# chrished/DEMC.jl

Hardware: AMD Instinct MI355X
Metric: chain-updates/sec (N x gens/s) + gens-to-Rhat<1.05, MvNormal d=5 N=1024 (higher is better)
Workload: dtype f64

## Files before the change

### demc.jl_amd/_lib.py

```python
from __future__ import annotations

import ctypes as C
import os
import subprocess
from pathlib import Path

import numpy as np

PKG_DIR = Path(__file__).resolve().parent
REPO_ROOT = PKG_DIR.parent
LIB_PATH = Path(os.environ["DEMCZ_LIB"]) if os.environ.get("DEMCZ_LIB") else PKG_DIR / "libdemcz_hip.so"
ABI_VERSION = 1
LAYOUT_SPLIT = 100
LAYOUT_SPLIT_WAVE = 164
LAYOUT_PROGRAM_WAVE = 264

TARGET_MVNORMAL, TARGET_ISO_QUAD, TARGET_LINREG_SSE, TARGET_HOST_CALLBACK, TARGET_PROGRAM = 0, 1, 2, 3, 4
OK, ERR_INVALID_ARGUMENT, ERR_HIP, ERR_CAPACITY, ERR_STATE, ERR_NO_DEVICE, ERR_COMM = range(7)

_dp = C.POINTER(C.c_double)
_ip = C.POINTER(C.c_int32)
_lp = C.POINTER(C.c_int64)

SYMBOLS = [
    "demcz_abi_version", "demcz_create", "demcz_destroy", "demcz_last_error", "demcz_set_state",
    "demcz_get_state", "demcz_set_history_origin", "demcz_run", "demcz_synchronize",
    "demcz_get_history", "demcz_get_changed", "demcz_rhat", "demcz_accept_ratio", "demcz_mean_cov",
    "demcz_propose", "demcz_accept_commit", "demcz_end_generation", "demcz_comm_unique_id",
    "demcz_comm_init", "demcz_export_current_device", "demcz_append_rows_device",
    "demcz_set_external_append", "demcz_get_info", "demcz_selftest_draws", "demcz_append_rows",
    "demcz_rhat_partial", "demcz_set_rng_offset", "demcz_rhat_array", "demcz_accept_ratio_array",
    "demcz_mean_cov_array", "demcz_set_append_lag", "demcz_run_checked", "demcz_set_kernel_timing",
    "demcz_get_kernel_time", "demcz_set_live_spin_limit", "demcz_get_live_status",
    "demcz_debug_append_slab", "demcz_get_changed_total", "demcz_debug_set_live_fault",
    "demcz_set_comm_timeout", "demcz_debug_stall_exchange", "demcz_get_kernel_time_series",
    "demcz_history_stream", "demcz_get_history_view", "demcz_detach_history", "demcz_release_host_buffer", "demcz_get_archive_pinned",
    "demcz_debug_kernel_counts", "demcz_pool_trim", "demcz_debug_kernel_name", "demcz_peer_group", "demcz_get_peer_status", "demcz_peer_export", "demcz_peer_attach",
    "demcz_peer_detach", "demcz_get_peer_ping", "demcz_set_live_rearms", "demcz_get_live_rearms",
    "demcz_closure_buffers", "demcz_program_check", "demcz_set_program",
    "demcz_program_check_layout",
]


class DemczError(RuntimeError):
    def __init__(self, code: int, msg: str):
        super().__init__(f"libdemcz_hip status {code}: {msg}")
        self.code = code


class Config(C.Structure):
    _fields_ = [
        ("N", C.c_int64), ("chain_id0", C.c_int64), ("d", C.c_int32), ("K", C.c_int32),
        ("Mcap", C.c_int64), ("Gcap", C.c_int64), ("Nblocks", C.c_int32),
        ("block_offsets", _ip), ("block_indices", _ip), ("eps_scale", _dp),
        ("seed", C.c_uint64), ("device_id", C.c_int32), ("target_kind", C.c_int32),
        ("mu", _dp), ("W", _dp), ("c0", C.c_double), ("design", _dp), ("yobs", _dp),
        ("nobs", C.c_int64), ("stream", C.c_void_p), ("lanes_per_chain", C.c_int32),
        ("reserved0", C.c_int32),
    ]


HIPCC_FLAGS = ["-O3", "--offload-arch=gfx950", "-ffp-contract=off", "-fPIC", "-Werror", "-Wno-pass-failed"]


def sources() -> list:
    csrc = PKG_DIR / "csrc"
    return ([csrc / "demcz_capi.hip"] + sorted(csrc.glob("demcz_pw_inst_*.hip")) + sorted(csrc.glob("demcz_mlr_inst_*.hip"))
            + [csrc / "demcz_program.hip"])


def build_command(out: Path = LIB_PATH) -> list:
    return ["hipcc"] + HIPCC_FLAGS + ["-shared", "-o", str(out)] + [str(p) for p in sources()] + ["-lrccl", "-lhiprtc"]


def build_lib(out: Path = LIB_PATH, extra: list = (), jobs: int = 0) -> Path:
    from concurrent.futures import ThreadPoolExecutor
    objdir = REPO_ROOT / "build" / "obj" / Path(out).stem
    objdir.mkdir(parents=True, exist_ok=True)
    srcs = sources()
    jobs = jobs or max(1, min(len(srcs), len(os.sched_getaffinity(0))))

    def compile_one(src):
        obj = objdir / (src.stem + ".o")
        r = subprocess.run(["hipcc"] + list(extra) + HIPCC_FLAGS + ["-c", "-o", str(obj), str(src)], capture_output=True, text=True)
        if r.returncode != 0:
            raise RuntimeError(f"hipcc failed on {src.name}:\n{r.stderr[-4000:]}")
        return obj

    with ThreadPoolExecutor(max_workers=jobs) as ex:
        objs = list(ex.map(compile_one, srcs))
    subprocess.run(["hipcc", "--offload-arch=gfx950", "-shared", "-fPIC", "-o", str(out)] + [str(o) for o in objs] + ["-lrccl", "-lhiprtc"], check=True)
    return Path(out)


def build(force: bool = False) -> Path:
    srcs = list((PKG_DIR / "csrc").glob("*")) + [REPO_ROOT / "include" / "demcz.h"]
    if not force and LIB_PATH.exists():
        newest = max(p.stat().st_mtime for p in srcs)
        if LIB_PATH.stat().st_mtime >= newest:
            return LIB_PATH
    return build_lib(LIB_PATH)


_LIB = None


def load():
    global _LIB
    if _LIB is not None:
        return _LIB
    if not LIB_PATH.exists():
        raise FileNotFoundError(
            f"{LIB_PATH} is missing: build it with `python -c 'import __graft_entry__ as g; g.build()'` "
            "(hipcc --offload-arch=gfx950).  There is no CPU fallback.")
    L = C.CDLL(str(LIB_PATH))
    L.demcz_abi_version.restype = C.c_int32
    if L.demcz_abi_version() != ABI_VERSION:
        raise RuntimeError("libdemcz_hip.so ABI version mismatch: rebuild")
    L.demcz_last_error.restype = C.c_char_p
    L.demcz_last_error.argtypes = [C.c_void_p]
    L.demcz_create.argtypes = [C.POINTER(C.c_void_p), C.POINTER(Config)]
    L.demcz_destroy.argtypes = [C.c_void_p]
    L.demcz_set_state.argtypes = [C.c_void_p, _dp, _dp, _dp, C.c_int64, C.c_int64]
    L.demcz_get_state.argtypes = [C.c_void_p, _dp, _dp, _dp, C.c_int64, _lp]
    L.demcz_set_history_origin.argtypes = [C.c_void_p, C.c_int64]
    L.demcz_run.argtypes = [C.c_void_p, C.c_int64, C.c_int64, C.c_double, _dp]
    L.demcz_synchronize.argtypes = [C.c_void_p]
    L.demcz_get_history.argtypes = [C.c_void_p, C.c_int64, C.c_int64, _dp, _dp]
    L.demcz_get_changed.argtypes = [C.c_void_p, C.c_int64, C.c_int64, _lp]
    L.demcz_get_changed_total.argtypes = [C.c_void_p, C.c_int64, C.c_int64, _lp, _ip]
    L.demcz_rhat.argtypes = [C.c_void_p, C.c_int64, C.c_int64, _dp]
    L.demcz_accept_ratio.argtypes = [C.c_void_p, C.c_int64, C.c_int64, _dp]
    L.demcz_mean_cov.argtypes = [C.c_void_p, C.c_int64, C.c_int64, _dp, _dp]
    L.demcz_propose.argtypes = [C.c_void_p, C.c_int64, C.c_int32, C.c_double, _dp]
    L.demcz_accept_commit.argtypes = [C.c_void_p, _dp, _dp]
    L.demcz_end_generation.argtypes = [C.c_void_p, C.c_int64]
    L.demcz_closure_buffers.argtypes = [C.c_void_p, C.POINTER(C.c_void_p), C.POINTER(C.c_void_p)]
    L.demcz_comm_unique_id.argtypes = [C.c_void_p]
    L.demcz_comm_init.argtypes = [C.c_void_p, C.c_void_p, C.c_int32, C.c_int32]
    L.demcz_export_current_device.argtypes = [C.c_void_p, C.c_void_p]
    L.demcz_append_rows_device.argtypes = [C.c_void_p, C.c_void_p, C.c_int64, C.c_int64]
    L.demcz_append_rows.argtypes = [C.c_void_p, _dp, C.c_int64, C.c_int64]
    L.demcz_rhat_partial.argtypes = [C.c_void_p, C.c_int64, C.c_int64, C.c_int32, _dp, _dp]
    L.demcz_set_rng_offset.argtypes = [C.c_void_p, C.c_int64]
    L.demcz_set_append_lag.argtypes = [C.c_void_p, C.c_int32]
    L.demcz_rhat_array.argtypes = [C.c_int32, _dp, C.c_int64, C.c_int32, C.c_int64, _dp]
    L.demcz_accept_ratio_array.argtypes = [C.c_int32, _dp, C.c_int64, C.c_int64, _dp]
    L.demcz_mean_cov_array.argtypes = [C.c_int32, _dp, C.c_int64, C.c_int32, C.c_int64, _dp, _dp]
    L.demcz_set_external_append.argtypes = [C.c_void_p, C.c_int32]
    L.demcz_get_info.argtypes = [C.c_void_p, _lp, _lp, _ip]
    L.demcz_selftest_draws.argtypes = [C.c_int32, C.c_uint64, C.c_uint64, C.c_uint64, C.c_int32,
                                       C.POINTER(C.c_uint64), _dp, _dp]
    L.demcz_set_live_spin_limit.argtypes = [C.c_void_p, C.c_int32]
    L.demcz_get_live_status.argtypes = [C.c_void_p, _ip, _ip]
    L.demcz_debug_kernel_counts.argtypes = [C.c_void_p, _lp]
    L.demcz_history_stream.argtypes = [C.c_void_p, C.c_int32]
    L.demcz_get_history_view.argtypes = [C.c_void_p, C.c_int64, C.c_int64, C.POINTER(C.c_void_p), C.POINTER(C.c_void_p)]
    L.demcz_detach_history.argtypes = [C.c_void_p, C.POINTER(C.c_void_p), C.POINTER(C.c_void_p)]
    L.demcz_release_host_buffer.argtypes = [C.c_void_p]
    L.demcz_pool_trim.argtypes = [_lp, _lp]
    L.demcz_peer_group.argtypes = [C.POINTER(C.c_void_p), C.c_int32]
    L.demcz_get_peer_status.argtypes = [C.c_void_p, _ip, _ip]
    L.demcz_peer_export.argtypes = [C.c_void_p, C.c_int32, C.c_int32, C.c_void_p]
    L.demcz_peer_attach.argtypes = [C.c_void_p, C.c_void_p]
    L.demcz_peer_detach.argtypes = [C.c_void_p]
    L.demcz_get_peer_ping.argtypes = [C.c_void_p, _ip, _dp]
    L.demcz_set_live_rearms.argtypes = [C.c_void_p, C.c_int32]
    L.demcz_get_live_rearms.argtypes = [C.c_void_p, _ip, _ip]
    L.demcz_debug_kernel_name.argtypes = [C.c_void_p, C.c_char_p, C.c_int32]
    L.demcz_program_check.argtypes = [C.c_int32, C.c_char_p, C.c_char_p]
    L.demcz_program_check_layout.argtypes = [C.c_int32, C.c_char_p, C.c_char_p, C.c_int32]
    L.demcz_set_program.argtypes = [C.c_void_p, C.c_char_p, C.c_char_p, _dp, C.c_int64]
    L.demcz_get_archive_pinned.argtypes = [C.c_void_p, C.POINTER(C.c_void_p), _lp]
    L.demcz_get_kernel_time_series.argtypes = [C.c_void_p, C.c_int32, _dp, _dp, _ip]
    L.demcz_set_comm_timeout.argtypes = [C.c_void_p, C.c_int64]
    L.demcz_debug_stall_exchange.argtypes = [C.c_void_p, C.c_int32]
    L.demcz_debug_set_live_fault.argtypes = [C.c_void_p, C.c_int32, C.c_int64]
    L.demcz_debug_append_slab.argtypes = [C.c_void_p, _dp, C.c_int32, C.c_int32, C.c_int32]
    for name in SYMBOLS:
        fn = getattr(L, name)
        if name != "demcz_last_error":
            fn.restype = C.c_int32
    _LIB = L
    return L


def f64(a, order="C"):
    return np.require(a, dtype=np.float64, requirements=["F" if order == "F" else "C", "A"])


def ptr(a, t=_dp):
    return a.ctypes.data_as(t) if a is not None else None
```

### demc.jl_amd/csrc/demcz_capi.hip

```cpp
#include "../../include/demcz.h"
#include "demcz_kernels.h"
#include "demcz_kernels_ml.h"
#include "demcz_kernels_pc.h"
#include "demcz_kernels_lr.h"
#include "demcz_kernels_ps.h"
#include "demcz_kernels_ps2.h"
#include "demcz_kernels_ps2d.h"
#include "demcz_pw_dispatch.h"
#include "demcz_mlr_dispatch.h"
#include "demcz_program.h"

#include <rccl/rccl.h>

#include <algorithm>
#include <chrono>
#include <thread>
#include <cstdlib>
#include <deque>
#include <mutex>
#include <cmath>
#include <cstdio>
#include <cstring>
#include <string>
#include <unordered_map>
// ... 123 lines not shown
    bool steady = false;
    KernelArm arm = ARM_ONE_LANE;
    bool live = false, temper = false;
    int pw_form = 0;
};

struct LaunchFacts {
    bool live = false;
    bool temper = false;
    bool ps2 = false;
    bool dual = false;
    bool pw_reg = false;
    bool pw_matrix = false;
    bool coop = false;
    bool lr16 = false;
};

struct PeerGroup {
    std::vector<demcz_handle*> members;
    bool failed = false;
    int32_t rearms_left = 3;
    bool lockstep_only = false;
    bool busy = false;
    bool dead = false;
};

struct demcz_handle {
    demcz_config cfg{};
    int lanes = 1;
    hipStream_t stream = nullptr;
    bool own_stream = false;
    std::string err;
    std::vector<int32_t> block_offsets, block_indices, slot_of;
    std::vector<double> eps;
    int64_t S = 0;
    int64_t ZS = 0;
    bool full_block = false;
    int ngrp = 1;
    uint64_t gstart = 1ull;
    int mlb_qb = 0;
    double* dZ = nullptr;
    double* dX = nullptr;
    double* dlp = nullptr;
    double* dchain = nullptr;
    double* dchain_alloc = nullptr;
    double* dlogobj = nullptr;
    double* dlp_origin = nullptr;
    bool origin_valid = false;
    double* dtemp = nullptr;
    int64_t temp_cap = 0;
    int32_t* d_block_offsets = nullptr;
    int32_t* d_slot_of = nullptr;
    double* d_eps = nullptr;
    double* d_mu = nullptr;
    double* d_Wp = nullptr;
    double* d_design = nullptr;
    double* d_y = nullptr;
    double* d_scratch = nullptr;
    int64_t scratch_cap = 0;
    double* d_stage = nullptr;
    int64_t stage_cap = 0;
    int64_t M = 0;
    int64_t g_done = 0;
    int64_t g0 = 0;
    int64_t rng_offset = 0;
    bool has_state = false;
    int64_t launches = 0;
    mutable int64_t kernel_counts[1] = {0};
    WindowKernel last_kernel;
    bool external_append = false;
    double* dXprop = nullptr;
    double* dlogu = nullptr;
    bool proposal_pending = false;
    bool gen_open = false;
    double* hc_X = nullptr;
    double* hc_lp = nullptr;
    volatile unsigned int* hc_flag = nullptr;
    unsigned int* hc_count = nullptr;
    unsigned int hc_seq = 0;
    hipStream_t diag_stream = nullptr;
    hipEvent_t diag_ev = nullptr;
    hipEvent_t rhat_side_ev = nullptr;
    bool rhat_side_pending = false;
    double* d_spec_X = nullptr;
    double* d_spec_lp = nullptr;
    hipEvent_t spec_ev = nullptr;
    double* pinned_rhat = nullptr;
    unsigned int* pinned_err = nullptr;
    int64_t pinned_err_launches = -1;
    int64_t pinned_cap = 0;
    bool timing = false;
    std::vector<std::pair<hipEvent_t, hipEvent_t>> timed;
    std::vector<double> series_start_ms, series_dur_ms;
    int64_t timed_launches = 0;
    int64_t live_wg_cap = -1;
    SplitKind split_kind = SPLIT_NONE;
    int split_lanes = 0;
    int split_per_wg = 1;
    int32_t* d_slot_role = nullptr;
    double* d_rec[2] = {nullptr, nullptr};
    unsigned int* d_live_err = nullptr;
#ifdef DEMCZ_STAMPS
    unsigned long long* d_stamps = nullptr;
#endif
    bool arena = false, rec_in_arena = false, hist_joint = false;
    int64_t arena_gens = 0;
    double* arena_rec[2] = {nullptr, nullptr};
    double* arena_temp = nullptr;
    int64_t rec_cap = 0;
    int rec_cur = 0;
    bool host_paced = false;
    int wpw = 1;
    bool ps_dual = false;
    bool dual_now = false;
    bool lr_spec = false;
    bool no_live = false;
    bool live_claimed = false;
    unsigned int live_spin_limit = 0;
    int32_t live_fault_polls = 0;
    int64_t live_fault_g = 0;
    bool in_checked = false;
    struct RunCall { int64_t g_from, g_to; double gamma; bool tempered; std::vector<double> temperature; };
    std::vector<RunCall> live_log;
    double* d_safe_X = nullptr;
    double* d_safe_lp = nullptr;
    bool snap_pending = false;
    int64_t safe_M = 0, safe_M_app = 0, safe_g_done = 0;
    bool replaying = false;
    int32_t live_redos = 0;
    int32_t live_rearms_left = 3;
    int32_t live_rearms = 0;
    int64_t rearm_from = -1;
    uint32_t fail_row_hint = 0xffffffffu;
    struct RecDesc { bool valid = false; int64_t g_first = 0, M = 0, rows = 0; int32_t ngen = 0, boff = 0; } rec_desc[2];
    hipStream_t prod_stream = nullptr;
    hipEvent_t prod_done[2] = {nullptr, nullptr};
    hipEvent_t prod_gate = nullptr;
    bool prod_pending[2] = {false, false};
    hipEvent_t after_launch_ev = nullptr;
    unsigned int* d_acc = nullptr;
    int64_t acc_waves = 0;
    int32_t acc_slots = 0, acc_next = 0;
    struct LaunchRec { int64_t g_first, g_last; int32_t slot; };
    std::deque<LaunchRec> acc_log;
    ncclComm_t comm = nullptr;
    ncclComm_t comm_side = nullptr;
    int nranks = 1, rank = 0;
    double* d_gather = nullptr;
    int lag = 0;
    int64_t M_app = 0;
    struct PendingRows { int64_t visible_from; int64_t M_after; hipEvent_t ev; int64_t xseq = 0; };
    std::deque<PendingRows> pending;
    int64_t batch_J = -1;
    hipStream_t comm_stream = nullptr;
    double* d_send[2] = {nullptr, nullptr};
    double* d_recv[2] = {nullptr, nullptr};
    hipEvent_t buf_done[2] = {nullptr, nullptr};
    int64_t xseq = 0, xseq_waited = 0, buf_xseq[2] = {0, 0};
    int batch_buf = 0, batch_cnt = 0;
    int64_t batch_base = 0;
    bool hs_on = false;
    double* hs_chain = nullptr;
    double* hs_logobj = nullptr;
    hipStream_t hs_stream = nullptr;
    bool pooled_dev = false;
    volatile long long* xdone = nullptr;
// ... 673 lines not shown
        for (int r = 0; r < DEMCZ_MAX_PEERS; ++r)
            if (h->ipc_mapped[r]) { (void)hipIpcCloseMemHandle(h->ipc_mapped[r]); h->ipc_mapped[r] = nullptr; }
        if (met) {
            met = false;
            if (ncclAllReduce(h->d_err_all + 1, h->d_err_all + 1, 1, ncclUint32, ncclMax, h->comm, h->stream) == ncclSuccess)
                met = sync_stream(h, h->stream, "demcz_destroy (peers, mappings closed)") == DEMCZ_OK;
        }
        if (!met && h->archive_fine) h->dZ = nullptr;
    }
    h->n_peers = 0;
    h->peer_mode = 0;
}

extern "C" int32_t demcz_destroy(demcz_handle* h)
{
    if (!h) return DEMCZ_OK;
    (void)hipSetDevice(h->cfg.device_id);
    for (hipStream_t st : {h->stream, h->prod_stream, h->diag_stream, h->comm_stream, h->hs_stream})
        if (st && !h->comm_dead) (void)sync_stream(h, st, "demcz_destroy");
    peer_detach(h);
    live_release(h);
    free_all(h);
    delete h;
    return DEMCZ_OK;
}

static TargetParams target_params(const demcz_handle* h)
{
    TargetParams tp;
    tp.mu = h->d_mu; tp.Wp = h->d_Wp; tp.c0 = h->cfg.c0;
    tp.design = h->d_design; tp.yobs = h->d_y; tp.nobs = h->cfg.nobs;
    tp.ngrp = h->ngrp; tp.goff = h->d_block_offsets; tp.gstart = h->gstart;
    return tp;
}

static int32_t ensure_scratch(demcz_handle* h, int64_t n)
{
    if (n <= h->scratch_cap) return DEMCZ_OK;
    { int32_t rcq = quiesce_all(h); if (rcq) return rcq; }
    SYNCCHK(h, h->stream);
    if (h->diag_stream) SYNCCHK(h, h->diag_stream);
    if (h->prod_stream) SYNCCHK(h, h->prod_stream);
    if (h->d_scratch) HIPCHK(h, dev_free(h->cfg.device_id, h->d_scratch));
    h->d_scratch = nullptr; h->scratch_cap = 0;
    HIPCHK(h, dev_malloc(h->cfg.device_id, (void**)&h->d_scratch, (size_t)n * sizeof(double)));
    h->scratch_cap = n;
    return DEMCZ_OK;
}

static int32_t launch_logp(demcz_handle* h, const double* X, int64_t ldX, int64_t n, double* out)
{
    const TargetParams tp = target_params(h);
    const int bs = 64;
    const dim3 grid((unsigned)((n + bs - 1) / bs));
    switch (h->cfg.target_kind) {
    case DEMCZ_TARGET_MVNORMAL:
        hipLaunchKernelGGL(logp_kernel<TARGET_MVNORMAL>, grid, dim3(bs), 0, h->stream, tp, h->cfg.d, X, ldX, n, out); break;
    case DEMCZ_TARGET_ISO_QUAD:
        hipLaunchKernelGGL(logp_kernel<TARGET_ISO_QUAD>, grid, dim3(bs), 0, h->stream, tp, h->cfg.d, X, ldX, n, out); break;
    case DEMCZ_TARGET_LINREG_SSE:
        hipLaunchKernelGGL(logp_kernel<TARGET_LINREG_SSE>, grid, dim3(bs), 0, h->stream, tp, h->cfg.d, X, ldX, n, out); break;
    case DEMCZ_TARGET_PROGRAM: {
        if (!h->prog_ready) return fail(h, DEMCZ_ERR_STATE, "program target: call demcz_set_program first");
        TargetParams tpv = tp;
        int dv = h->cfg.d;
        void* args[] = {&tpv, &dv, &X, &ldX, &n, &out};
        HIPCHK(h, hipModuleLaunchKernel(h->prog.logp, grid.x, 1, 1, bs, 1, 1, 0, h->stream, args, nullptr));
        break;
    }
    default: return fail(h, DEMCZ_ERR_STATE, "host-callback target: pass logp explicitly");
    }
    HIPCHK(h, hipGetLastError());
    return DEMCZ_OK;
}

extern "C" int32_t demcz_set_state(demcz_handle* h, const double* X, const double* logp, const double* Z,
                                   int64_t ldZ, int64_t M0)
{
    if (!h) return DEMCZ_ERR_INVALID_ARGUMENT;
    DEADCHK(h);
    if (!X || !Z) return fail(h, DEMCZ_ERR_INVALID_ARGUMENT, "demcz_set_state: X and Z are required");
    if (M0 < 2) return fail(h, DEMCZ_ERR_INVALID_ARGUMENT, "demcz_set_state: M0 >= 2 needed (two distinct archive rows, demcz.jl:176-179)");
    if (M0 > h->cfg.Mcap || ldZ < M0) return fail(h, DEMCZ_ERR_CAPACITY, "demcz_set_state: M0 exceeds Mcap or ldZ < M0");
    if (!logp && h->cfg.target_kind == DEMCZ_TARGET_HOST_CALLBACK)
        return fail(h, DEMCZ_ERR_INVALID_ARGUMENT, "demcz_set_state: host-callback target needs logp");
    if (h->cfg.target_kind == DEMCZ_TARGET_PROGRAM && !h->prog_ready)
        return fail(h, DEMCZ_ERR_STATE, "demcz_set_state: program target: call demcz_set_program first");
    HIPCHK(h, hipSetDevice(h->cfg.device_id));
    const int d = h->cfg.d;
    const int64_t N = h->cfg.N;
    HIPCHK(h, hipMemcpyAsync(h->dX, X, (size_t)N * d * sizeof(double), hipMemcpyHostToDevice, h->stream));
    {
        int32_t rcz = ensure_scratch(h, M0 * d);
        if (rcz) return rcz;
        HIPCHK(h, hipMemcpy2DAsync(h->d_scratch, (size_t)M0 * sizeof(double), Z, (size_t)ldZ * sizeof(double),
                                   (size_t)M0 * sizeof(double), (size_t)d, hipMemcpyHostToDevice, h->stream));
        const int64_t tot = M0 * d;
        hipLaunchKernelGGL(append_rows_kernel, dim3((unsigned)((tot + 255) / 256)), dim3(256), 0, h->stream, h->dZ, h->ZS,
                           (int64_t)0, (const double*)h->d_scratch, M0, M0, d);
        HIPCHK(h, hipGetLastError());
        const size_t rest = (size_t)(h->cfg.Mcap - M0) * (size_t)h->ZS;
        if (rest > 0) {
            hipLaunchKernelGGL(fill_u64_kernel, dim3((unsigned)((rest + 255) / 256)), dim3(256), 0, h->stream,
                               reinterpret_cast<unsigned long long*>(h->dZ + (size_t)M0 * h->ZS), rest, LIVE_SENTINEL);
            HIPCHK(h, hipGetLastError());
        }
        HIPCHK(h, hipMemsetAsync(h->d_live_err, 0, 4 * sizeof(unsigned int), h->stream));
    }
    if (logp) {
        HIPCHK(h, hipMemcpyAsync(h->dlp, logp, (size_t)N * sizeof(double), hipMemcpyHostToDevice, h->stream));
    } else {
        int32_t rc = launch_logp(h, h->dX, N, N, h->dlp);
        if (rc) return rc;
    }
    HIPCHK(h, hipMemcpyAsync(h->dlp_origin, h->dlp, (size_t)N * sizeof(double), hipMemcpyDeviceToDevice, h->stream));
    SYNCCHK(h, h->stream);
    h->M = M0;
    h->M_app = M0;
    h->peer_fence = true;
    if (h->no_live && h->rearm_from >= 0) h->rearm_from = 0;
    h->live_log.clear();
    h->snap_pending = false;
    h->acc_log.clear();
    { int32_t rcs = rec_scrub(h); if (rcs) return rcs; }
    for (auto& pe : h->pending) if (pe.ev) (void)hipEventDestroy(pe.ev);
    h->pending.clear();
    h->batch_cnt = 0; h->batch_J = -1;
    h->g_done = h->g0;
    h->origin_valid = true;
    h->has_state = true;
    h->proposal_pending = false;
    h->gen_open = false;
    return DEMCZ_OK;
}

extern "C" int32_t demcz_get_state(demcz_handle* h, double* X, double* logp, double* Z, int64_t ldZ, int64_t* M)
{
    if (!h) return DEMCZ_ERR_INVALID_ARGUMENT;
    DEADCHK(h);
    if (!h->has_state) return fail(h, DEMCZ_ERR_STATE, "demcz_get_state: no state set");
    HIPCHK(h, hipSetDevice(h->cfg.device_id));
    {
        int32_t rcv = live_verify(h);
        if (rcv) return rcv;
    }
    const int d = h->cfg.d;
    const int64_t N = h->cfg.N;
    if (X) HIPCHK(h, hipMemcpyAsync(X, h->dX, (size_t)N * d * sizeof(double), hipMemcpyDeviceToHost, h->stream));
    if (logp) HIPCHK(h, hipMemcpyAsync(logp, h->dlp, (size_t)N * sizeof(double), hipMemcpyDeviceToHost, h->stream));
    if (Z) {
        const int64_t Mall = h->M_app;
        if (ldZ < Mall) return fail(h, DEMCZ_ERR_INVALID_ARGUMENT, "demcz_get_state: ldZ < M");
        int32_t rcz = flush_exchanges(h);
        if (rcz) return rcz;
        rcz = ensure_scratch(h, Mall * d);
        if (rcz) return rcz;
        const int64_t tot = Mall * d;
        hipLaunchKernelGGL(export_rows_kernel, dim3((unsigned)((tot + 255) / 256)), dim3(256), 0, h->stream, (const double*)h->dZ,
                           h->ZS, (int64_t)0, h->d_scratch, Mall, Mall, d);
        HIPCHK(h, hipGetLastError());
        HIPCHK(h, hipMemcpy2DAsync(Z, (size_t)ldZ * sizeof(double), h->d_scratch, (size_t)Mall * sizeof(double),
                                   (size_t)Mall * sizeof(double), (size_t)d, hipMemcpyDeviceToHost, h->stream));
    }
    SYNCCHK(h, h->stream);
    if (M) *M = h->M_app;
    return DEMCZ_OK;
// ... 111 lines not shown
    if (h->cfg.target_kind == DEMCZ_TARGET_PROGRAM && !h->prog_ready)
        return fail(h, DEMCZ_ERR_STATE, "demcz_run: program target: call demcz_set_program first");
    if (!k.fn && !k.mod) return fail(h, DEMCZ_ERR_STATE, "window launch: target / dimension not built for this handle's layout");
    void* args[] = {const_cast<WindowParams*>(&P)};
    if (k.mod) {
        HIPCHK(h, hipModuleLaunchKernel(k.mod, (unsigned)blocks, 1, 1, (unsigned)k.threads, 1, 1, (unsigned)k.dyn_lds, h->stream, args, nullptr));
    } else {
        allow_dynamic_lds(h->cfg.device_id, k);
        HIPCHK(h, hipLaunchKernel(k.fn, dim3((unsigned)blocks), dim3((unsigned)k.threads), args, k.dyn_lds, h->stream));
    }
    HIPCHK(h, hipGetLastError());
    if (k.steady) ++h->kernel_counts[0];
    return DEMCZ_OK;
}

static int ml_lanes_available(int target_kind, int d, bool full_block, int64_t nobs, int max_blocklen = 0, int nblocks = 1)
{
    if (!full_block) {
        if (nblocks > MLB_MAX_BLOCKS) return 0;
        if (target_kind == DEMCZ_TARGET_MVNORMAL) {
            if ((d == 5 || d == 6 || d == 10) && 2 + (max_blocklen + 1) / 2 <= 8) return 8;
            if (d == 20 && 2 + (max_blocklen + 1) / 2 <= 16) return 16;
        }
        return 0;
    }
    if (target_kind == DEMCZ_TARGET_LINREG_SSE && d == 10 &&
        lr16_dynamic_lds<10>(nobs) <= ML_MAX_DYNAMIC_LDS)
        return 16;
    if (target_kind == DEMCZ_TARGET_LINREG_SSE && d >= 2 && d <= 28) return 16;
    if (target_kind == DEMCZ_TARGET_MVNORMAL) {
        if (d >= 2 && d <= 10) return 8;
        if (d == 20) return 16;
    }
    if (target_kind == DEMCZ_TARGET_ISO_QUAD && d == 10) return 8;
    return 0;
}

static bool mlb32_wanted(int64_t)
{
    static const char* env = getenv("DEMCZ_MLB_L32");
    return env && atoi(env) != 0;
}

static bool pc_available(int target_kind, int d, bool full_block)
{
    if (!full_block) return false;
    if (target_kind == DEMCZ_TARGET_ISO_QUAD) return d == 10;
    return target_kind == DEMCZ_TARGET_MVNORMAL && d >= 2 && d <= 10;
}

static bool split_ml_available(int target_kind, int d, bool full_block, int64_t nobs)
{
    if (!full_block) return false;
    if (target_kind == DEMCZ_TARGET_MVNORMAL) return d == 20;
    return target_kind == DEMCZ_TARGET_LINREG_SSE && d == 10 && lr16_dynamic_lds<10>(nobs) <= ML_MAX_DYNAMIC_LDS;
}

static bool ps_available(int target_kind, int d)
{
    if (target_kind == DEMCZ_TARGET_MVNORMAL) return d >= 2 && d <= PW_D_MAX;
    return target_kind == DEMCZ_TARGET_ISO_QUAD && d >= PW_D_MIN && d <= PW_D_MAX;
}

static int pc_roles(int d) { return ((d == 1) ? 1 : (d + 1) / 2) + 2; }
static int64_t rec_fields(const demcz_handle* h) { return (h->split_kind == SPLIT_MLB) ? 2 * h->S : (int64_t)h->cfg.d + 2; }
static int64_t rec_roles(const demcz_handle* h) { return (h->split_kind == SPLIT_MLB) ? h->S : pc_roles(h->cfg.d); }

#ifdef DEMCZ_STAMPS
constexpr int64_t DEMCZ_STAMP_WGS = 1 << 16;
#endif

static bool pw_matrix_form(const demcz_handle* h)
{
    const char* on = getenv("DEMCZ_PW_MFMA");
    return on && atoi(on) != 0 && h->cfg.d == 20 && h->cfg.target_kind == DEMCZ_TARGET_MVNORMAL;
}

static bool pw_regular(const WindowParams& P, bool live)
{
    static const bool no_reg = getenv("DEMCZ_NO_PW_REG") != nullptr;
    return live && !no_reg && P.K % PS_R == 0 && P.to_boundary % PS_R == 0 && P.ngen % PS_R == 0 && P.ngen >= PS_R;
}

static int32_t launch_window_pc(demcz_handle* h, const WindowParams& P, const WindowKernel& k, bool live = false)
{
    const int64_t nbc = (P.N + 63) / 64;
    const bool pc_records = !(h->split_kind == SPLIT_MLB);
    const int64_t units = pc_records ? produce_units(P.N, (int)rec_roles(h), P.rec_fields, P.next_ngen) : nbc * rec_roles(h) * P.next_ngen;
    const int upw = k.waves;
    const int64_t blocks = P.consumer_blocks + (units + upw - 1) / upw;
    if (blocks <= 0) return DEMCZ_OK;
    if (h->split_kind == SPLIT_WAVE || h->lr_spec) {
        if (h->split_kind == SPLIT_WAVE && P.ZS != ((P.d <= 2) ? 2 : (P.d <= 4) ? 4 : ((P.d + 7) / 8) * 8)) return fail(h, DEMCZ_ERR_STATE, "split layout: archive row stride");
        const int bin = (P.rec_in == h->d_rec[0]) ? 0 : 1, bout = (P.rec_out == h->d_rec[0]) ? 0 : 1;
        const bool one_launch = !live && P.consumer_blocks > 0;
        if (units > 0 && one_launch && h->prod_pending[bout]) {
            HIPCHK(h, hipStreamWaitEvent(h->stream, h->prod_done[bout], 0));
            h->prod_pending[bout] = false;
        }
        if (units > 0 && !one_launch) {
            hipStream_t ps = h->stream;
            static const bool serial_env = getenv("DEMCZ_PRODUCE_SERIAL") != nullptr;
            if (P.consumer_blocks > 0 && !serial_env && h->peer_mode != 1) {
                if (!h->prod_stream) {
                    HIPCHK(h, stream_acquire(h->cfg.device_id, &h->prod_stream));
                    HIPCHK(h, hipEventCreateWithFlags(&h->prod_gate, hipEventDisableTiming));
                    for (int b = 0; b < 2; ++b) HIPCHK(h, hipEventCreateWithFlags(&h->prod_done[b], hipEventDisableTiming));
                }
                if (h->after_launch_ev) {
                    HIPCHK(h, hipStreamWaitEvent(h->prod_stream, h->after_launch_ev, 0));
                } else {
                    HIPCHK(h, hipEventRecord(h->prod_gate, h->stream));
                    HIPCHK(h, hipStreamWaitEvent(h->prod_stream, h->prod_gate, 0));
                }
                ps = h->prod_stream;
            } else if (h->prod_pending[bout]) {
                HIPCHK(h, hipStreamWaitEvent(h->stream, h->prod_done[bout], 0));
                h->prod_pending[bout] = false;
            }
            const dim3 pg((unsigned)((units + PRODUCE_WAVES - 1) / PRODUCE_WAVES)), pw(64 * PRODUCE_WAVES);
            static const size_t throttle_env = getenv("DEMCZ_PRODUCE_LDS") ? (size_t)atol(getenv("DEMCZ_PRODUCE_LDS")) : PRODUCE_THROTTLE_LDS;
            size_t big_d = throttle_env;
            if (h->split_kind == SPLIT_WAVE && P.d > 20) {
                int plds = 0;
                if (h->prog_wave && (!h->prog_ready || hipFuncGetAttribute(&plds, HIP_FUNC_ATTRIBUTE_SHARED_SIZE_BYTES, h->prog.wave[1][0]) != hipSuccess)) plds = (int)ML_MAX_DYNAMIC_LDS;
                size_t clds = (size_t)plds;
                if (!h->prog_wave) {
                    WindowKernel lk[MAX_LIVE_KERNELS];
                    const int nlk = live_kernels(h, lk);
                    for (int i = 0; i < nlk; ++i) {
                        hipFuncAttributes a{};
                        if (lk[i].fn && hipFuncGetAttributes(&a, lk[i].fn) == hipSuccess) clds = std::max(clds, (size_t)a.sharedSizeBytes);
                    }
                }
                const size_t room = (clds + 4096 < ML_MAX_DYNAMIC_LDS) ? ML_MAX_DYNAMIC_LDS - clds - 4096 : 8192;
                big_d = std::max<size_t>(8192, std::min<size_t>(throttle_env, room));
            }
            const size_t dyn = (ps != h->stream) ? (h->lr_spec ? (size_t)8192 : (h->ps_dual && !getenv("DEMCZ_PRODUCE_LDS")) ? (size_t)32768 : big_d) : 0;
            switch (P.d) {
#define DEMCZ_PRODUCE_CASE(DD) case DD: hipLaunchKernelGGL((produce_kernel<DD>), pg, pw, dyn, ps, P); break;
            DEMCZ_PRODUCE_CASE(2) DEMCZ_PRODUCE_CASE(3) DEMCZ_PRODUCE_CASE(4) DEMCZ_PRODUCE_CASE(5) DEMCZ_PRODUCE_CASE(6) DEMCZ_PRODUCE_CASE(7)
            DEMCZ_PRODUCE_CASE(8) DEMCZ_PRODUCE_CASE(9) DEMCZ_PRODUCE_CASE(10) DEMCZ_PRODUCE_CASE(11) DEMCZ_PRODUCE_CASE(12) DEMCZ_PRODUCE_CASE(13)
            DEMCZ_PRODUCE_CASE(14) DEMCZ_PRODUCE_CASE(15) DEMCZ_PRODUCE_CASE(16) DEMCZ_PRODUCE_CASE(17) DEMCZ_PRODUCE_CASE(18) DEMCZ_PRODUCE_CASE(19)
            DEMCZ_PRODUCE_CASE(20) DEMCZ_PRODUCE_CASE(21) DEMCZ_PRODUCE_CASE(22) DEMCZ_PRODUCE_CASE(23) DEMCZ_PRODUCE_CASE(24) DEMCZ_PRODUCE_CASE(25)
            DEMCZ_PRODUCE_CASE(26) DEMCZ_PRODUCE_CASE(27) DEMCZ_PRODUCE_CASE(28) DEMCZ_PRODUCE_CASE(29) DEMCZ_PRODUCE_CASE(30) DEMCZ_PRODUCE_CASE(31)
            DEMCZ_PRODUCE_CASE(32)
#undef DEMCZ_PRODUCE_CASE
            default: return fail(h, DEMCZ_ERR_STATE, "split layout: dimension not built");
            }
            HIPCHK(h, hipGetLastError());
            if (ps != h->stream) {
                HIPCHK(h, hipEventRecord(h->prod_done[bout], ps));
                h->prod_pending[bout] = true;
            }
        }
        if (P.consumer_blocks > 0) {
            if (h->prod_pending[bin]) {
                if (h->host_paced) { int32_t rcw = sync_event(h, h->prod_done[bin], "launch_window_pc"); if (rcw) return rcw; }
                else HIPCHK(h, hipStreamWaitEvent(h->stream, h->prod_done[bin], 0));
                h->prod_pending[bin] = false;
            }
            static_assert(PS_CHAINS == LR16_WAVES, "producer units per workgroup of a one-launch grid");
            const int64_t grid = P.consumer_blocks + (one_launch ? (units + PS_CHAINS - 1) / PS_CHAINS : 0);
            return launch_kernel(h, k, grid, P);
        }
        return DEMCZ_OK;
    }
    return launch_kernel(h, k, blocks, P);
}

static int32_t rec_reserve(demcz_handle* h, int64_t gens)
{
    if (gens <= h->rec_cap) return DEMCZ_OK;
    { int32_t rcq = quiesce_all(h); if (rcq) return rcq; }
    SYNCCHK(h, h->stream);
    if (h->prod_stream) SYNCCHK(h, h->prod_stream);
    h->prod_pending[0] = h->prod_pending[1] = false;
    if (h->arena && gens <= h->arena_gens && h->rec_cap == 0) {
        for (int b = 0; b < 2; ++b) { h->d_rec[b] = h->arena_rec[b]; h->rec_desc[b].valid = false; }
        h->rec_in_arena = true;
        h->rec_cap = h->arena_gens;
        return DEMCZ_OK;
    }
    for (int b = 0; b < 2; ++b) {
        if (h->d_rec[b] && !h->rec_in_arena) HIPCHK(h, dev_free(h->cfg.device_id, h->d_rec[b]));
        h->d_rec[b] = nullptr;
        const size_t nd = (size_t)gens * (size_t)rec_fields(h) * h->cfg.N + REC_PAD;
        HIPCHK(h, dev_malloc(h->cfg.device_id, (void**)&h->d_rec[b], nd * sizeof(double)));
        HIPCHK(h, hipMemsetAsync(h->d_rec[b], 0, nd * sizeof(double), h->stream));
        h->rec_desc[b].valid = false;
    }
    h->rec_in_arena = false;
    h->rec_cap = gens;
    return DEMCZ_OK;
}

static bool ps2_applicable(const demcz_handle* h, const WindowParams& P)
{
    static const bool off = getenv("DEMCZ_NO_PS2") != nullptr;
    if (off || h->split_kind != SPLIT_WAVE || h->prog_wave || P.d < 2 || P.d > 5 || !h->arena || !h->rec_in_arena) return false;
    if (P.temperature && (P.temperature < h->arena_temp || P.temperature >= h->arena_temp + h->arena_gens)) return false;
    if (P.K % PS2_R != 0 || P.to_boundary % PS2_R != 0 || P.ngen % PS2_R != 0 || P.ngen < PS2_R) return false;
    if (P.chain && (!h->hist_joint || (double)h->cfg.N * (h->cfg.d + 1) * (double)h->cfg.Gcap * 8.0 >= 4293918720.0)) return false;
    return true;
}

static int32_t pc_prepare(demcz_handle* h, WindowParams& P, int64_t cur_rows, int64_t next_g, int64_t next_ngen, int64_t next_M,
                          int64_t next_rows, int32_t next_boff)
{
    {
        int32_t rcr = rec_reserve(h, std::max<int64_t>(P.ngen, next_ngen));
        if (rcr) return rcr;
    }
    P.rec_stride = h->rec_cap;
    const int cur = h->rec_cur;
    const int32_t cur_boff = P.K - P.to_boundary;
    auto& dc = h->rec_desc[cur];
    if (!(dc.valid && dc.g_first == P.g_first && dc.ngen >= P.ngen && dc.M == P.M && dc.rows == cur_rows && dc.boff == cur_boff)) {
        WindowParams Q = P;
        Q.consumer_blocks = 0;
        Q.rec_out = h->d_rec[cur];
        Q.next_g_first = P.g_first; Q.next_ngen = P.ngen; Q.next_M = P.M; Q.next_rows = cur_rows; Q.next_boff = cur_boff;
        int32_t rc = launch_window_pc(h, Q, window_kernel_of(h, launch_facts(h, &Q, false)));
        if (rc) return rc;
        dc.valid = true; dc.g_first = P.g_first; dc.M = P.M; dc.ngen = P.ngen; dc.rows = cur_rows; dc.boff = cur_boff;
    }
    P.rec_in = h->d_rec[cur];
    const int per_wg = (h->ps_dual && !h->dual_now) ? PS_CHAINS : h->split_per_wg;
    P.consumer_blocks = (int32_t)((P.N + per_wg - 1) / per_wg);
    P.rec_out = h->d_rec[cur ^ 1];
    P.next_g_first = next_g; P.next_ngen = (int32_t)std::max<int64_t>(next_ngen, 0); P.next_M = next_M;
    P.next_rows = next_rows; P.next_boff = next_boff;
    auto& dn = h->rec_desc[cur ^ 1];
    dn.valid = next_ngen > 0; dn.g_first = next_g; dn.M = next_M; dn.ngen = (int32_t)std::max<int64_t>(next_ngen, 0);
    dn.rows = next_rows; dn.boff = next_boff;
    h->rec_cur = cur ^ 1;
// ... 282 lines not shown
    if (h->batch_cnt == 0) return DEMCZ_OK;
    const int d = h->cfg.d, cnt = h->batch_cnt, buf = h->batch_buf;
    const int64_t N = h->cfg.N;
    hipEvent_t ready;
    HIPCHK(h, hipEventCreateWithFlags(&ready, hipEventDisableTiming));
    HIPCHK(h, hipEventRecord(ready, h->stream));
    HIPCHK(h, hipStreamWaitEvent(h->comm_stream, ready, 0));
    HIPCHK(h, hipEventDestroy(ready));
    { int32_t rcs = maybe_stall(h, h->comm_stream); if (rcs) return rcs; }
    NCCLCHK(h, ncclAllGather(h->d_send[buf], h->d_recv[buf], (size_t)N * d * cnt, ncclDouble, h->comm_side, h->comm_stream));
    const int64_t tot = N * d * cnt * h->nranks;
    hipLaunchKernelGGL(append_batch_kernel, dim3((unsigned)((tot + 255) / 256)), dim3(256), 0, h->comm_stream, h->dZ, h->ZS,
                       h->batch_base, (const double*)h->d_recv[buf], N, h->nranks, cnt, d);
    HIPCHK(h, hipGetLastError());
    hipEvent_t done;
    HIPCHK(h, hipEventCreateWithFlags(&done, hipEventDisableTiming));
    HIPCHK(h, hipEventRecord(done, h->comm_stream));
    h->pending.back().ev = done;
    h->pending.back().xseq = ++h->xseq;
    if (!h->xdone) {
        HIPCHK(h, host_malloc((void**)&h->xdone, sizeof(long long)));
        *h->xdone = 0;
    }
    hipLaunchKernelGGL(mark_kernel, dim3(1), dim3(1), 0, h->comm_stream, h->xdone, (long long)h->xseq);
    HIPCHK(h, hipGetLastError());
    h->buf_xseq[buf] = h->xseq;
    HIPCHK(h, hipEventRecord(h->buf_done[buf], h->comm_stream));
    h->batch_cnt = 0;
    h->batch_buf ^= 1;
    h->batch_J = -1;
    return DEMCZ_OK;
}

static int32_t admit_pending(demcz_handle* h, int64_t g)
{
    while (!h->pending.empty() && h->pending.front().visible_from <= g) {
        auto pe = h->pending.front();
        if (pe.ev) {
            if (h->host_paced && h->xdone) {
                volatile long long* xd = h->xdone;
                const long long need = (long long)pe.xseq;
                int32_t rcw = wait_deadline(h, [xd, need]() { return (*xd >= need) ? hipSuccess : hipErrorNotReady; }, "admit_pending (exchange of a batch)");
                if (rcw) return rcw;
            }
            else HIPCHK(h, hipStreamWaitEvent(h->stream, pe.ev, 0));
            HIPCHK(h, hipEventDestroy(pe.ev));
            h->xseq_waited = std::max(h->xseq_waited, pe.xseq);
        }
        h->M = pe.M_after;
        h->pending.pop_front();
    }
    return DEMCZ_OK;
}

static int32_t flush_exchanges(demcz_handle* h)
{
    if (h->comm && h->lag > 0) {
        int32_t rc = exchange_batch(h);
        if (rc) return rc;
        for (auto& pe : h->pending)
            if (pe.ev) HIPCHK(h, hipStreamWaitEvent(h->stream, pe.ev, 0));
    }
    return DEMCZ_OK;
}

static int32_t check_live_err(demcz_handle* h)
{
    unsigned int e[4] = {0, 0, 0, 0};
    if (!h->d_live_err) return DEMCZ_OK;
    if (h->err_clean) return DEMCZ_OK;
    HIPCHK(h, hipMemcpy(e, h->d_live_err, sizeof(e), hipMemcpyDeviceToHost));
    if (!e[0]) h->err_clean = true;
    if (e[0])
        return fail(h, DEMCZ_ERR_HIP, "demcz_run: an archive row appended inside the launch never became visible (LIVE hand-off): "
                                      "generation " + std::to_string(e[1]) + " of the launch, row " + std::to_string(e[2]) +
                                      ", workgroup " + std::to_string(e[3]) + ", rows appended " + std::to_string(h->M_app));
    return DEMCZ_OK;
}

static int32_t live_rollback(demcz_handle* h, std::vector<demcz_handle::RunCall>& calls)
{
    calls.swap(h->live_log);
    h->live_log.clear();
    const int64_t N = h->cfg.N;
    const int d = h->cfg.d;
    SYNCCHK(h, h->stream);
    if (h->diag_stream) SYNCCHK(h, h->diag_stream);
    if (h->prod_stream) SYNCCHK(h, h->prod_stream);
    if (!h->snap_pending) {
        HIPCHK(h, hipMemcpyAsync(h->dX, h->d_safe_X, (size_t)N * d * sizeof(double), hipMemcpyDeviceToDevice, h->stream));
        HIPCHK(h, hipMemcpyAsync(h->dlp, h->d_safe_lp, (size_t)N * sizeof(double), hipMemcpyDeviceToDevice, h->stream));
    }
    h->snap_pending = false;
    if (h->M_app > h->safe_M_app) {
        const size_t rest = (size_t)(h->M_app - h->safe_M_app) * (size_t)h->ZS;
        hipLaunchKernelGGL(fill_u64_kernel, dim3((unsigned)((rest + 255) / 256)), dim3(256), 0, h->stream,
                           reinterpret_cast<unsigned long long*>(h->dZ + (size_t)h->safe_M_app * h->ZS), rest, LIVE_SENTINEL);
        HIPCHK(h, hipGetLastError());
    }
    HIPCHK(h, hipMemsetAsync(h->d_live_err, 0, 4 * sizeof(unsigned int), h->stream));
    SYNCCHK(h, h->stream);
    h->peer_fence = true;
    int64_t from = h->g_done;
    if (h->fail_row_hint != 0xffffffffu && (int64_t)h->fail_row_hint >= h->safe_M_app && (int64_t)h->fail_row_hint < h->M_app) {
        const int64_t rows = h->cfg.N * ((h->comm || h->peer_mode != 0) ? h->nranks : 1);
        const int64_t j = ((int64_t)h->fail_row_hint - h->safe_M_app) / rows;
        from = std::min<int64_t>(from, (h->safe_g_done / h->cfg.K + 1 + j) * (int64_t)h->cfg.K + 1);
    }
    h->fail_row_hint = 0xffffffffu;
    h->M = h->safe_M;
    h->M_app = h->safe_M_app;
    h->g_done = h->safe_g_done;
    while (!h->acc_log.empty() && h->acc_log.back().g_last > h->safe_g_done) h->acc_log.pop_back();
    { int32_t rcs = rec_scrub(h); if (rcs) return rcs; }
    h->no_live = true;
    h->rearm_from = -1;
    if (h->peer_mode != 1 && h->peer_mode != 3 && h->live_rearms_left > 0) {
        --h->live_rearms_left;
        h->rearm_from = from;
    }
    h->live_fault_polls = 0;
    live_release(h);
    ++h->live_redos;
    return DEMCZ_OK;
}

static int32_t live_try_rearm(demcz_handle* h)
{
    h->rearm_from = -1;
    h->no_live = false;
    unsigned int ok = live_span(h) > 0 ? 1u : 0u;
    if (h->peer_mode == 2 && h->comm && h->d_err_all) {
        HIPCHK(h, hipMemcpyAsync(h->d_err_all + 2, &ok, sizeof(ok), hipMemcpyHostToDevice, h->stream));
        NCCLCHK(h, ncclAllReduce(h->d_err_all + 2, h->d_err_all + 2, 1, ncclUint32, ncclMin, h->comm, h->stream));
        SYNCCHK(h, h->stream);
        HIPCHK(h, hipMemcpy(&ok, h->d_err_all + 2, sizeof(ok), hipMemcpyDeviceToHost));
    }
    if (!ok) {
        h->no_live = true;
        live_release(h);
        return DEMCZ_OK;
    }
    ++h->live_rearms;
    if (getenv("DEMCZ_DEBUG_LIVE")) fprintf(stderr, "[demcz] rank %d: LIVE launches re-armed (%d re-arms left)\n", h->rank, (int)h->live_rearms_left);
    return DEMCZ_OK;
}

static int32_t live_failed(demcz_handle* h, bool& failed)
{
    failed = false;
    SYNCCHK(h, h->stream);
    unsigned int e[4] = {0, 0, 0, 0};
    if (h->peer_mode == 2 && !h->no_live && h->comm) {
        NCCLCHK(h, ncclAllReduce(h->d_live_err, h->d_err_all, 1, ncclUint32, ncclMax, h->comm, h->stream));
        SYNCCHK(h, h->stream);
        HIPCHK(h, hipMemcpy(e, h->d_err_all, sizeof(unsigned int), hipMemcpyDeviceToHost));
    } else if (h->pinned_err && h->pinned_err_launches == h->launches) {
        std::memcpy(e, h->pinned_err, sizeof(e));
    } else {
        HIPCHK(h, hipMemcpy(e, h->d_live_err, sizeof(e), hipMemcpyDeviceToHost));
    }
    h->pinned_err_launches = -1;
    failed = e[0] != 0u;
    if (!failed && h->peer_mode != 2) h->err_clean = true;
    if (failed) {
        unsigned int row = 0xffffffffu;
// ... 322 lines not shown

extern "C" int32_t demcz_run(demcz_handle* h, int64_t g_from, int64_t g_to, double gamma, const double* temperature)
{
    if (!h) return DEMCZ_ERR_INVALID_ARGUMENT;
    DEADCHK(h);
    if (!h->has_state) return fail(h, DEMCZ_ERR_STATE, "demcz_run: call demcz_set_state first");
    if (g_from < 1 || g_to < g_from) return fail(h, DEMCZ_ERR_INVALID_ARGUMENT, "demcz_run: need 1 <= g_from <= g_to");
    if (h->cfg.target_kind == DEMCZ_TARGET_HOST_CALLBACK)
        return fail(h, DEMCZ_ERR_STATE, "demcz_run: host-callback target uses demcz_propose/accept_commit");
    const bool hist = h->cfg.Gcap > 0;
    if (hist && (g_from - h->g0 - 1 < 0 || g_to - h->g0 > h->cfg.Gcap))
        return fail(h, DEMCZ_ERR_CAPACITY, "demcz_run: generations outside the history window (demcz_set_history_origin)");
    HIPCHK(h, hipSetDevice(h->cfg.device_id));
    const int64_t G = g_to - g_from + 1;
    const int K = h->cfg.K;
    const bool sharded = (h->comm != nullptr);
    if (h->peer_mode == 1 && (!h->group || h->group->dead))
        return fail(h, DEMCZ_ERR_STATE, "demcz_run: a member of this handle's replica group has been destroyed");
    if (h->no_live && h->rearm_from >= 0 && g_from > h->rearm_from) {
        int32_t rcr = live_try_rearm(h);
        if (rcr) return rcr;
    }
    const bool peer = h->peer_mode != 0 && live_span(h) > 0;
    const bool rccl_exchange = sharded && !peer;
    const bool kernel_appends = !rccl_exchange && !h->external_append;
    const int64_t shards = (sharded || h->peer_mode != 0) ? h->nranks : 1;
    {
        const int64_t nb = g_to / K - (g_from - 1) / K;
        const int64_t rows = h->cfg.N * shards;
        if (!h->external_append && h->M_app + nb * rows > h->cfg.Mcap)
            return fail(h, DEMCZ_ERR_CAPACITY, "demcz_run: Z row capacity (Mcap) would be exceeded");
        if (h->external_append && nb > 1)
            return fail(h, DEMCZ_ERR_STATE, "demcz_run: with external append a call may cross at most one K boundary, at its end");
        if (h->external_append && nb == 1 && (g_to % K) != 0)
            return fail(h, DEMCZ_ERR_STATE, "demcz_run: with external append the K boundary must be the last generation of the call");
    }
    if (h->peer_mode == 3 && h->peers_closed)
        return fail(h, DEMCZ_ERR_STATE, "demcz_run: the peers' archives have been closed (demcz_peer_detach): this handle runs no further generations");
    if (h->peer_mode == 3 && !peer)
        return fail(h, DEMCZ_ERR_STATE, "demcz_run: host-mediated IPC peers run with the in-launch hand-off only (it is not available: a timed-out "
                                        "hand-off, an append lag, caller-owned appends, or more chains than a LIVE launch holds)");
    if (h->peer_mode == 1 && !peer && !h->replaying) {
        if (h->lag != 0 || h->external_append) return fail(h, DEMCZ_ERR_STATE, "demcz_run: replica groups run with append lag 0 and library-owned appends");
        demcz_handle::RunCall rcall{g_from, g_to, gamma, temperature != nullptr, {}};
        if (temperature) rcall.temperature.assign(temperature, temperature + G);
        h->live_log.push_back(std::move(rcall));
        return DEMCZ_OK;
    }
    const bool temp_in_arena = temperature && h->arena && h->arena_temp && G <= h->arena_gens;
    if (temperature && temp_in_arena) {
        SYNCCHK(h, h->stream);
        HIPCHK(h, hipMemcpyAsync(h->arena_temp, temperature, (size_t)G * sizeof(double), hipMemcpyHostToDevice, h->stream));
        SYNCCHK(h, h->stream);
    } else if (temperature) {
        if (G > h->temp_cap) {
            { int32_t rcq = quiesce_all(h); if (rcq) return rcq; }
            SYNCCHK(h, h->stream);
            if (h->dtemp) HIPCHK(h, dev_free(h->cfg.device_id, h->dtemp));
            h->dtemp = nullptr; h->temp_cap = 0;
            HIPCHK(h, dev_malloc(h->cfg.device_id, (void**)&h->dtemp, (size_t)(G + 8) * sizeof(double)));
            HIPCHK(h, hipMemsetAsync(h->dtemp, 0, (size_t)(G + 8) * sizeof(double), h->stream));
            h->temp_cap = G;
        }
        HIPCHK(h, hipMemcpyAsync(h->dtemp, temperature, (size_t)G * sizeof(double), hipMemcpyHostToDevice, h->stream));
        SYNCCHK(h, h->stream);
    }
    WindowParams P;
    P.Z = h->dZ; P.Zw = h->dZ; P.ZS = h->ZS;
    P.Xcur = h->dX; P.lpcur = h->dlp;
    P.chain = hist ? h->dchain : nullptr; P.logobj = hist ? h->dlogobj : nullptr;
#ifdef DEMCZ_EXP_NOHIST
    P.chain = nullptr; P.logobj = nullptr;
#endif
    P.N = h->cfg.N; P.chain_id0 = h->cfg.chain_id0; P.d = h->cfg.d;
    P.gamma = gamma; P.seed = h->cfg.seed; P.S = h->S; P.Nblocks = h->cfg.Nblocks;
    P.block_offsets = h->d_block_offsets; P.slot_of = h->d_slot_of; P.eps = h->d_eps; P.slot_role = h->d_slot_role;
    P.tp = target_params(h);
    P.snap = nullptr;
    P.K = K;
    P.acc_out = nullptr; P.live_err = h->d_live_err; P.live_spin_limit = LIVE_SPIN_LIMIT;
    P.safe_X = nullptr; P.safe_lp = nullptr;
    P.rec_in = nullptr; P.rec_out = nullptr; P.next_g_first = 0; P.next_M = 0; P.next_ngen = 0; P.consumer_blocks = 0;
    P.next_rows = 0; P.next_boff = 0; P.rec_stride = 0;
    P.rec_fields = (h->lanes == DEMCZ_LAYOUT_SPLIT && h->split_kind == SPLIT_ML) ? h->cfg.d + 2 : 0;
    P.z_bytes = (uint32_t)std::min<size_t>(h->dZ_bytes, 0xffffffffull);
    P.hist_bytes = (hist && h->hist_joint) ? (uint32_t)std::min<double>((double)h->cfg.N * (h->cfg.d + 1) * (double)h->cfg.Gcap * 8.0, 4294967295.0) : 0u;
    P.brows = h->cfg.N * (peer ? shards : 1);
    P.row_off = peer ? (int64_t)h->rank * h->cfg.N : 0;
    P.n_peers = peer ? h->n_peers : 0;
    for (int r = 0; r < DEMCZ_MAX_PEERS; ++r) P.peer_Z[r] = (peer && r < h->n_peers) ? h->peer_Z[r] : nullptr;
    if (peer && h->peer_mode == 2 && h->peer_fence) {
        NCCLCHK(h, ncclAllReduce(h->d_err_all + 1, h->d_err_all + 1, 1, ncclUint32, ncclMax, h->comm, h->stream));
        h->peer_fence = false;
    }
#ifdef DEMCZ_STAMPS
    if (!h->d_stamps) {
        HIPCHK(h, dev_malloc(h->cfg.device_id, (void**)&h->d_stamps, (size_t)DEMCZ_STAMP_WGS * 16 * sizeof(unsigned long long)));
        HIPCHK(h, hipMemset(h->d_stamps, 0, (size_t)DEMCZ_STAMP_WGS * 16 * sizeof(unsigned long long)));
    }
    P.stamps = h->d_stamps;
#endif
    const int E = h->lag;
    int64_t g = g_from;
    if (h->lanes == DEMCZ_LAYOUT_SPLIT) {
        const int64_t lm = live_span(h);
        int64_t cap = (lm > 0) ? lm : (int64_t)K * std::max(E, 1);
        if (lm > 0 && hist) cap = std::max<int64_t>(std::min<int64_t>(cap, h->cfg.Gcap), std::min<int64_t>(cap, G));
        int32_t rcr = rec_reserve(h, cap);
        if (rcr) return rcr;
    }
    if (live_span(h) > 0) {
        if (h->live_log.size() >= 256 && !h->in_checked && !h->replaying && h->peer_mode != 1) {
            int32_t rcv = live_verify(h);
            if (rcv) return rcv;
        }
        if (live_span(h) > 0) {
            if (h->live_log.empty() && !h->replaying) {
                const int64_t N = h->cfg.N;
                const int d = h->cfg.d;
                if (!h->d_safe_X) HIPCHK(h, dev_malloc(h->cfg.device_id, (void**)&h->d_safe_X, (size_t)N * d * sizeof(double)));
                if (!h->d_safe_lp) HIPCHK(h, dev_malloc(h->cfg.device_id, (void**)&h->d_safe_lp, (size_t)N * sizeof(double)));
                if (h->live_fault_polls < 0) {
                    HIPCHK(h, hipMemsetAsync(h->d_safe_X, 0xff, (size_t)N * d * sizeof(double), h->stream));
                    HIPCHK(h, hipMemsetAsync(h->d_safe_lp, 0xff, (size_t)N * sizeof(double), h->stream));
                }
                h->snap_pending = true;
                h->safe_M = h->M; h->safe_M_app = h->M_app; h->safe_g_done = h->g_done;
            }
            demcz_handle::RunCall rcall{g_from, g_to, gamma, temperature != nullptr, {}};
            if (temperature) rcall.temperature.assign(temperature, temperature + G);
            h->live_log.push_back(std::move(rcall));
        }
    }
    struct EventPair {
        hipEvent_t a = nullptr, b = nullptr;
        ~EventPair() { if (a) (void)hipEventDestroy(a); if (b) (void)hipEventDestroy(b); }
    } tev;
    int64_t timed_launches = 0;
    const bool timed = h->timing && h->timed.size() < 4096;
    if (timed) {
        HIPCHK(h, hipEventCreate(&tev.a));
        HIPCHK(h, hipEventCreate(&tev.b));
        HIPCHK(h, hipEventRecord(tev.a, h->stream));
    }
    while (g <= g_to) {
        const int64_t next_boundary = ((g - 1) / K + 1) * K;
        int64_t w_end = std::min(next_boundary, g_to);
        if (E > 0 && !h->external_append) {
            const int64_t jn = next_boundary / K, J = ((jn + E - 1) / E) * E;
            w_end = std::min(J * (int64_t)K, g_to);
        }
        int64_t live_max = live_span(h);
        h->dual_now = false;
        if (h->ps_dual) {
            const int64_t tb0 = next_boundary - g + 1, rest = g_to - g + 1;
            const bool temp_ok = !temperature || temp_in_arena;
            const bool hist_ok = !hist || (double)h->cfg.N * (h->cfg.d + 1) * (double)h->cfg.Gcap * 8.0 < 4293918720.0;
            const bool reg = K % PS2_R == 0 && tb0 % PS2_R == 0 && rest >= PS2_R && temp_ok && hist_ok && h->arena && h->rec_in_arena;
            if (reg) {
                h->dual_now = true;
                if (live_max > 0) live_max = std::max<int64_t>((std::min(live_max, rest) / PS2_R) * PS2_R, PS2_R);
                else w_end = g + ((w_end - g + 1) / PS2_R) * PS2_R - 1;
            } else {
                live_max = 0;
            }
        }
// ... 208 lines not shown
        if (first >= 0 && r.g_last == g_to) { last = i; break; }
    }
    bool ok = first >= 0 && last >= first;
    for (int i = first; ok && i < last; ++i)
        ok = h->acc_log[i].g_last + 1 == h->acc_log[i + 1].g_first && (h->acc_log[i].slot + 1) % h->acc_slots == h->acc_log[i + 1].slot;
    if (ok && h->d_acc) {
        rc = ensure_scratch(h, 1);
        if (rc) return rc;
        static_assert(sizeof(long long) == sizeof(double), "scratch reuse");
        hipLaunchKernelGGL(sum_counts_kernel, dim3(1), dim3(256), 0, h->stream, (const unsigned int*)h->d_acc, h->acc_waves,
                           (int)h->acc_log[first].slot, last - first + 1, (int)h->acc_slots, skip, (long long*)h->d_scratch);
        HIPCHK(h, hipGetLastError());
        long long v = 0;
        HIPCHK(h, hipMemcpyAsync(&v, h->d_scratch, sizeof(v), hipMemcpyDeviceToHost, h->stream));
        SYNCCHK(h, h->stream);
        *total = (int64_t)v;
        if (from_ballots) *from_ballots = 1;
        return DEMCZ_OK;
    }
    std::vector<int64_t> ch((size_t)(g_to - g_from + 1));
    rc = demcz_get_changed(h, g_from, g_to, ch.data());
    if (rc) return rc;
    int64_t t = 0;
    for (int64_t v : ch) t += v;
    *total = t;
    if (from_ballots) *from_ballots = 0;
    return DEMCZ_OK;
}

struct RhatPlan { int64_t N, w, s0, n, nd; int d, nchunk; double *S1, *S2, *mean_j, *s2_j, *sums; };

static int32_t rhat_prepare(demcz_handle* h, int64_t g_from, int64_t g_to, RhatPlan& r, bool compute, hipStream_t qs = nullptr)
{
    int32_t rc = check_hist_range(h, g_from, g_to, "demcz_rhat");
    if (rc) return rc;
    r.N = h->cfg.N; r.w = g_to - g_from + 1; r.s0 = g_from - h->g0 - 1; r.d = h->cfg.d;
    r.n = r.w / 2;
    if (r.n < 2) return fail(h, DEMCZ_ERR_INVALID_ARGUMENT, "demcz_rhat: window needs at least 4 generations");
    HIPCHK(h, hipSetDevice(h->cfg.device_id));
    r.nchunk = (int)std::min<int64_t>(std::max<int64_t>(1, r.n / 32), 32);
    r.nd = r.N * r.d;
    const int64_t need = 2 * (2 * r.nchunk * r.nd) + 2 * (2 * r.nd) + 4 * r.d;
    rc = ensure_scratch(h, need);
    if (rc) return rc;
    r.S1 = h->d_scratch;
    r.S2 = r.S1 + 2 * r.nchunk * r.nd;
    r.mean_j = r.S2 + 2 * r.nchunk * r.nd;
    r.s2_j = r.mean_j + 2 * r.nd;
    r.sums = r.s2_j + 2 * r.nd;
    if (compute) {
        const int bs = 256;
        const unsigned gx = (unsigned)((r.nd + bs - 1) / bs);
        if (!qs) qs = h->stream;
        hipLaunchKernelGGL(rhat_moments_kernel, dim3(gx, 2 * r.nchunk), dim3(bs), 0, qs, h->dchain, r.N, r.d, r.s0, r.n, r.nchunk, r.S1, r.S2);
        hipLaunchKernelGGL(rhat_chainstats_kernel, dim3(gx, 2), dim3(bs), 0, qs, h->dchain, r.N, r.d, r.s0, r.n, r.nchunk, r.S1, r.S2, r.mean_j, r.s2_j);
        HIPCHK(h, hipGetLastError());
    }
    return DEMCZ_OK;
}

extern "C" int32_t demcz_rhat_partial(demcz_handle* h, int64_t g_from, int64_t g_to, int32_t stage, const double* grand, double* out)
{
    if (!h || !out || (stage != 0 && stage != 1) || (stage == 1 && !grand)) return DEMCZ_ERR_INVALID_ARGUMENT;
    RhatPlan r;
    int32_t rc = live_verify(h);
    if (rc) return rc;
    rc = rhat_prepare(h, g_from, g_to, r, true);
    if (rc) return rc;
    const int d = r.d;
    if (stage == 0) {
        hipLaunchKernelGGL(rhat_reduce_kernel, dim3(d), dim3(256), 0, h->stream, r.mean_j, r.s2_j, r.N, d, 0, (const double*)nullptr, 1.0, r.sums);
        HIPCHK(h, hipGetLastError());
        HIPCHK(h, hipMemcpyAsync(out, r.sums, (size_t)d * sizeof(double), hipMemcpyDeviceToHost, h->stream));
    } else {
        HIPCHK(h, hipMemcpyAsync(r.sums, grand, (size_t)d * sizeof(double), hipMemcpyHostToDevice, h->stream));
        hipLaunchKernelGGL(rhat_reduce_kernel, dim3(d), dim3(256), 0, h->stream, r.mean_j, r.s2_j, r.N, d, 1, (const double*)r.sums, 1.0, r.sums + d);
        HIPCHK(h, hipGetLastError());
        HIPCHK(h, hipMemcpyAsync(out, r.sums + d, (size_t)2 * d * sizeof(double), hipMemcpyDeviceToHost, h->stream));
    }
    SYNCCHK(h, h->stream);
    return DEMCZ_OK;
}

static int32_t rhat_enqueue(demcz_handle* h, int64_t g_from, int64_t g_to, double* out, bool side = false)
{
    RhatPlan r;
    hipStream_t qs = h->stream;
    static const bool own_env = getenv("DEMCZ_RHAT_OWN_STREAM") != nullptr;
    if (side && !h->comm && !own_env && h->prod_stream) {
        if (!h->diag_ev) HIPCHK(h, hipEventCreateWithFlags(&h->diag_ev, hipEventDisableTiming));
        if (h->after_launch_ev) {
            HIPCHK(h, hipStreamWaitEvent(h->prod_stream, h->after_launch_ev, 0));
        } else {
            HIPCHK(h, hipEventRecord(h->diag_ev, h->stream));
            HIPCHK(h, hipStreamWaitEvent(h->prod_stream, h->diag_ev, 0));
            h->after_launch_ev = h->diag_ev;
        }
        qs = h->prod_stream;
    } else if (side && h->comm && h->peer_mode == 2 && !h->no_live && h->comm_side && h->comm_stream && h->lag == 0) {
        if (!h->diag_ev) HIPCHK(h, hipEventCreateWithFlags(&h->diag_ev, hipEventDisableTiming));
        if (h->after_launch_ev) {
            HIPCHK(h, hipStreamWaitEvent(h->comm_stream, h->after_launch_ev, 0));
        } else {
            HIPCHK(h, hipEventRecord(h->diag_ev, h->stream));
            HIPCHK(h, hipStreamWaitEvent(h->comm_stream, h->diag_ev, 0));
            h->after_launch_ev = h->diag_ev;
        }
        qs = h->comm_stream;
    } else if (side && !h->comm) {
        if (!h->diag_stream) HIPCHK(h, stream_acquire(h->cfg.device_id, &h->diag_stream));
        if (!h->diag_ev) HIPCHK(h, hipEventCreateWithFlags(&h->diag_ev, hipEventDisableTiming));
        if (h->after_launch_ev) {
            HIPCHK(h, hipStreamWaitEvent(h->diag_stream, h->after_launch_ev, 0));
        } else {
            HIPCHK(h, hipEventRecord(h->diag_ev, h->stream));
            HIPCHK(h, hipStreamWaitEvent(h->diag_stream, h->diag_ev, 0));
            h->after_launch_ev = h->diag_ev;
        }
        qs = h->diag_stream;
    }
    if (qs == h->stream && h->rhat_side_pending) {
        HIPCHK(h, hipStreamWaitEvent(h->stream, h->rhat_side_ev, 0));
        h->rhat_side_pending = false;
    }
    struct SideMark {
        demcz_handle* h; hipStream_t qs;
        ~SideMark() {
            if (qs == h->stream) return;
            if (!h->rhat_side_ev && hipEventCreateWithFlags(&h->rhat_side_ev, hipEventDisableTiming) != hipSuccess) { h->rhat_side_ev = nullptr; return; }
            if (hipEventRecord(h->rhat_side_ev, qs) == hipSuccess) h->rhat_side_pending = true;
        }
    } side_mark{h, qs};
    int32_t rc = rhat_prepare(h, g_from, g_to, r, true, qs);
    if (rc) return rc;
    const int d = r.d;
    const int64_t n = r.n;
    const int64_t m = 2 * r.N * h->nranks;
    const bool sharded = (h->comm != nullptr);
    double* sums = r.sums;
    if (!sharded) {
        hipLaunchKernelGGL(rhat_tail_kernel, dim3(d), dim3(256), 0, qs, r.mean_j, r.s2_j, r.N, d, (double)n, (double)m, sums + 3 * d);
        HIPCHK(h, hipGetLastError());
        HIPCHK(h, hipMemcpyAsync(out, sums + 3 * d, (size_t)d * sizeof(double), hipMemcpyDeviceToHost, qs));
        return DEMCZ_OK;
    }
    const ncclComm_t cq = (qs == h->comm_stream && qs != h->stream) ? h->comm_side : h->comm;
    hipLaunchKernelGGL(rhat_reduce_kernel, dim3(d), dim3(256), 0, qs, r.mean_j, r.s2_j, r.N, d, 0, (const double*)nullptr, 1.0, sums);
    HIPCHK(h, hipGetLastError());
    NCCLCHK(h, ncclAllReduce(sums, sums, (size_t)d, ncclDouble, ncclSum, cq, qs));
    hipLaunchKernelGGL(rhat_reduce_kernel, dim3(d), dim3(256), 0, qs, r.mean_j, r.s2_j, r.N, d, 1, (const double*)sums, (double)m, sums + d);
    HIPCHK(h, hipGetLastError());
    NCCLCHK(h, ncclAllReduce(sums + d, sums + d, (size_t)2 * d, ncclDouble, ncclSum, cq, qs));
    hipLaunchKernelGGL(rhat_final_kernel, dim3((unsigned)((d + 63) / 64)), dim3(64), 0, qs, (const double*)(sums + d), d, (double)n, (double)m, sums + 3 * d);
    HIPCHK(h, hipGetLastError());
    HIPCHK(h, hipMemcpyAsync(out, sums + 3 * d, (size_t)d * sizeof(double), hipMemcpyDeviceToHost, qs));
    return DEMCZ_OK;
}

extern "C" int32_t demcz_rhat(demcz_handle* h, int64_t g_from, int64_t g_to, double* rhat)
{
    if (!h || !rhat) return DEMCZ_ERR_INVALID_ARGUMENT;
    int32_t rc = live_verify(h);
    if (rc) return rc;
    rc = rhat_enqueue(h, g_from, g_to, rhat);
    if (rc) return rc;
    SYNCCHK(h, h->stream);
    return DEMCZ_OK;
}

extern "C" int32_t demcz_accept_ratio(demcz_handle* h, int64_t g_from, int64_t g_to, double* ratio)
{
    if (!h || !ratio) return DEMCZ_ERR_INVALID_ARGUMENT;
    int32_t rc = check_hist_range(h, g_from, g_to, "demcz_accept_ratio");
    if (rc) return rc;
    const int64_t N = h->cfg.N, w = g_to - g_from + 1, s0 = g_from - h->g0 - 1;
    if (w < 2) return fail(h, DEMCZ_ERR_INVALID_ARGUMENT, "demcz_accept_ratio: need at least 2 generations");
    HIPCHK(h, hipSetDevice(h->cfg.device_id));
    rc = live_verify(h);
    if (rc) return rc;
    rc = ensure_scratch(h, 2 * N);
    if (rc) return rc;
    {
        const int64_t cb = (N + 63) / 64;
        const int nchunk = (int)std::max<int64_t>(1, std::min<int64_t>(std::min<int64_t>((w - 1 + 31) / 32, 1024), (4096 + cb - 1) / cb));
        unsigned int* cnt = reinterpret_cast<unsigned int*>(h->d_scratch + N);
        HIPCHK(h, hipMemsetAsync(cnt, 0, (size_t)N * sizeof(unsigned int), h->stream));
        hipLaunchKernelGGL(changed_per_chain_kernel, dim3((unsigned)cb, (unsigned)nchunk), dim3(64), 0, h->stream, h->dlogobj, N, s0, w, nchunk, cnt);
        hipLaunchKernelGGL(changed_ratio_kernel, dim3((unsigned)((N + 255) / 256)), dim3(256), 0, h->stream, (const unsigned int*)cnt, N, w, h->d_scratch);
    }
    HIPCHK(h, hipGetLastError());
    HIPCHK(h, hipMemcpyAsync(ratio, h->d_scratch, (size_t)N * sizeof(double), hipMemcpyDeviceToHost, h->stream));
    SYNCCHK(h, h->stream);
    return DEMCZ_OK;
}

extern "C" int32_t demcz_mean_cov(demcz_handle* h, int64_t g_from, int64_t g_to, double* mean, double* cov)
{
    if (!h || !mean || !cov) return DEMCZ_ERR_INVALID_ARGUMENT;
    int32_t rc = check_hist_range(h, g_from, g_to, "demcz_mean_cov");
    if (rc) return rc;
    const int64_t N = h->cfg.N, w = g_to - g_from + 1, s0 = g_from - h->g0 - 1;
    const int d = h->cfg.d;
    HIPCHK(h, hipSetDevice(h->cfg.device_id));
    rc = live_verify(h);
    if (rc) return rc;
    const int T = (d + MC_TS - 1) / MC_TS, npair = T * (T + 1) / 2;
    const int64_t cb = (N + 255) / 256;
    const int nchunk = (int)std::max<int64_t>(1, std::min<int64_t>(std::min<int64_t>((w + 15) / 16, 512), (2048 + cb * npair - 1) / (cb * npair)));
    const int64_t nblk_xy = cb * nchunk;
    rc = ensure_scratch(h, (int64_t)d * (d + 1) + d + nblk_xy * npair * MC_VALS);
    if (rc) return rc;
    double* sums = h->d_scratch;
    double* partial = sums + (int64_t)d * (d + 1) + d;
    hipLaunchKernelGGL(meancov_partial_kernel, dim3((unsigned)cb, (unsigned)nchunk, (unsigned)npair), dim3(256), 0, h->stream,
                       (const double*)h->dchain, N, d, s0, w, nchunk, partial);
    hipLaunchKernelGGL(meancov_final_kernel, dim3((unsigned)((d * (d + 1) + 63) / 64)), dim3(64), 0, h->stream, (const double*)partial, d,
                       (int)nblk_xy, sums);
    HIPCHK(h, hipGetLastError());
    std::vector<double> hs((size_t)d * (d + 1)), ref((size_t)d);
    HIPCHK(h, hipMemcpyAsync(hs.data(), sums, hs.size() * sizeof(double), hipMemcpyDeviceToHost, h->stream));
    HIPCHK(h, hipMemcpy2DAsync(ref.data(), sizeof(double), h->dchain + (size_t)N * d * s0, (size_t)N * sizeof(double),
                               sizeof(double), (size_t)d, hipMemcpyDeviceToHost, h->stream));
    SYNCCHK(h, h->stream);
    const double cnt = (double)(N * w);
    std::vector<double> dm((size_t)d);
    for (int p = 0; p < d; ++p) { dm[p] = hs[(size_t)p + (size_t)d * d] / cnt; mean[p] = ref[p] + dm[p]; }
    for (int p = 0; p < d; ++p)
        for (int q = 0; q < d; ++q) cov[p + d * q] = hs[(size_t)p + (size_t)d * q] / cnt - dm[p] * dm[q];
    return DEMCZ_OK;
}

namespace demcz {
__device__ __forceinline__ void propose_done(unsigned int* done_count, unsigned int* host_flag, unsigned int seq)
{
    if (!host_flag) return;
    __threadfence_system();
    __syncthreads();
    if (threadIdx.x == 0) {
// ... 759 lines not shown
        h->pinned_cap = cap;
    }
    double* pinned = h->pinned_rhat;
    auto max_of = [d](const double* r) {
        double mx = r[0];
        for (int p = 1; p < d; ++p) mx = (r[p] > mx || r[p] != r[p]) ? r[p] : mx;
        return mx;
    };
    int32_t rc = DEMCZ_OK;
    const bool speculate = !monitor && !h->comm && h->lag == 0 && !h->external_append && !temperature;
    const int64_t N = h->cfg.N;
    if (speculate) {
        if (!h->d_spec_X) HIPCHK(h, dev_malloc(h->cfg.device_id, (void**)&h->d_spec_X, (size_t)N * d * sizeof(double)));
        if (!h->d_spec_lp) HIPCHK(h, dev_malloc(h->cfg.device_id, (void**)&h->d_spec_lp, (size_t)N * sizeof(double)));
        if (!h->spec_ev) HIPCHK(h, hipEventCreateWithFlags(&h->spec_ev, hipEventDisableTiming));
    }
    bool ahead = false;
    while (g <= g_to && rc == DEMCZ_OK) {
        const int64_t nxt = std::min(g_to, ((g - 1) / every + 1) * every);
        if (!ahead) rc = demcz_run(h, g, nxt, gamma, temperature ? temperature + (g - g_from) : nullptr);
        ahead = false;
        if (rc) break;
        if (nxt % every == 0 && nxt - every >= h->g0) {
            double* slot = pinned + (size_t)checks * d;
            rc = rhat_enqueue(h, nxt - every + 1, nxt, slot, monitor && nxt < g_to);
            if (rc) break;
            ++checks;
            if (!monitor) {
                int64_t M_before = 0;
                if (speculate && nxt < g_to) {
                    if (hipEventRecord(h->spec_ev, h->stream) != hipSuccess) { rc = fail(h, DEMCZ_ERR_HIP, "demcz_run_checked: event failed"); break; }
                    if (hipMemcpyAsync(h->d_spec_X, h->dX, (size_t)N * d * sizeof(double), hipMemcpyDeviceToDevice, h->stream) != hipSuccess ||
                        hipMemcpyAsync(h->d_spec_lp, h->dlp, (size_t)N * sizeof(double), hipMemcpyDeviceToDevice, h->stream) != hipSuccess) {
                        rc = fail(h, DEMCZ_ERR_HIP, "demcz_run_checked: snapshot failed");
                        break;
                    }
                    M_before = h->M_app;
                    const int64_t nn = std::min(g_to, (nxt / every + 1) * every);
                    rc = demcz_run(h, nxt + 1, nn, gamma, nullptr);
                    if (rc) break;
                    ahead = true;
                    if ((rc = sync_event(h, h->spec_ev, "demcz_run_checked")) != DEMCZ_OK) break;
                } else if ((rc = sync_stream(h, h->stream, "demcz_run_checked")) != DEMCZ_OK) {
                    break;
                }
                if (max_of(slot) < threshold) {
                    if (g_stop) *g_stop = nxt;
                    if (ahead) {
                        if ((rc = sync_stream(h, h->stream, "demcz_run_checked")) != DEMCZ_OK) break;
                        rc = check_live_err(h);
                        if (rc) break;
                        if (hipMemcpyAsync(h->dX, h->d_spec_X, (size_t)N * d * sizeof(double), hipMemcpyDeviceToDevice, h->stream) != hipSuccess ||
                            hipMemcpyAsync(h->dlp, h->d_spec_lp, (size_t)N * sizeof(double), hipMemcpyDeviceToDevice, h->stream) != hipSuccess) {
                            rc = fail(h, DEMCZ_ERR_HIP, "demcz_run_checked: restore failed");
                            break;
                        }
                        const size_t rest = (size_t)(h->M_app - M_before) * (size_t)h->ZS;
                        if (rest > 0) {
                            hipLaunchKernelGGL(fill_u64_kernel, dim3((unsigned)((rest + 255) / 256)), dim3(256), 0, h->stream,
                                               reinterpret_cast<unsigned long long*>(h->dZ + (size_t)M_before * h->ZS), rest, LIVE_SENTINEL);
                            if (hipGetLastError() != hipSuccess) { rc = fail(h, DEMCZ_ERR_HIP, "demcz_run_checked: restore failed"); break; }
                        }
                        const int64_t s_lo = nxt - h->g0, s_hi = std::min<int64_t>(h->g_done - h->g0, h->cfg.Gcap);
                        if (s_hi > s_lo &&
                            (hipMemsetAsync(h->dchain + (size_t)N * d * s_lo, 0, (size_t)N * d * (s_hi - s_lo) * sizeof(double), h->stream) != hipSuccess ||
                             hipMemsetAsync(h->dlogobj + (size_t)N * s_lo, 0, (size_t)N * (s_hi - s_lo) * sizeof(double), h->stream) != hipSuccess)) {
                            rc = fail(h, DEMCZ_ERR_HIP, "demcz_run_checked: restore failed");
                            break;
                        }
                        if (h->hs_on) { h->after_launch_ev = nullptr; rc = stream_history(h, nxt + 1, h->g_done); if (rc) break; }
                        h->M_app = M_before;
                        h->M = M_before;
                        h->g_done = nxt;
                        if ((rc = rec_scrub(h)) != DEMCZ_OK) break;
                        if (!h->live_log.empty() && h->live_log.back().g_from == nxt + 1) h->live_log.pop_back();
                        while (!h->acc_log.empty() && h->acc_log.back().g_last > nxt) h->acc_log.pop_back();
                    }
                    break;
                }
            }
        }
        g = nxt + 1;
    }
    h->pinned_err_launches = -1;
    if (rc == DEMCZ_OK && !h->live_log.empty() && h->peer_mode != 2) {
        if (!h->pinned_err && host_malloc((void**)&h->pinned_err, 4 * sizeof(unsigned int)) != hipSuccess) { h->pinned_err = nullptr; (void)hipGetLastError(); }
        if (h->pinned_err && hipMemcpyAsync(h->pinned_err, h->d_live_err, 4 * sizeof(unsigned int), hipMemcpyDeviceToHost, h->stream) == hipSuccess)
            h->pinned_err_launches = h->launches;
    }
    if (rc == DEMCZ_OK) rc = sync_stream(h, h->stream, "demcz_run_checked");
    if (rc == DEMCZ_OK && h->diag_stream) rc = sync_stream(h, h->diag_stream, "demcz_run_checked");
    if (rc == DEMCZ_OK && h->prod_stream) rc = sync_stream(h, h->prod_stream, "demcz_run_checked");
    if (rc == DEMCZ_OK && h->comm_stream) rc = sync_stream(h, h->comm_stream, "demcz_run_checked");
    if (rc == DEMCZ_OK) {
        for (int32_t i = 0; i < checks; ++i)
            if (rhat_max && i < n_max) rhat_max[i] = max_of(pinned + (size_t)i * d);
        if (rhat_last && checks > 0) std::copy(pinned + (size_t)(checks - 1) * d, pinned + (size_t)checks * d, rhat_last);
        if (n_checks) *n_checks = checks;
    }
    return rc;
}

extern "C" int32_t demcz_run_checked(demcz_handle* h, int64_t g_from, int64_t g_to, double gamma, const double* temperature,
                                     int64_t every, double threshold, int64_t* g_stop, int32_t* n_checks,
                                     double* rhat_max, int32_t n_max, double* rhat_last)
{
    if (!h) return DEMCZ_ERR_INVALID_ARGUMENT;
    DEADCHK(h);
    if (every < 4 || g_from < 1 || g_to < g_from) return fail(h, DEMCZ_ERR_INVALID_ARGUMENT, "demcz_run_checked: need every >= 4 and 1 <= g_from <= g_to");
    if (!h->has_state) return fail(h, DEMCZ_ERR_STATE, "demcz_run_checked: call demcz_set_state first");
    if (h->peer_mode == 1 || h->peer_mode == 3) return fail(h, DEMCZ_ERR_STATE, "demcz_run_checked: replica groups and host-mediated peers are driven call by call (demcz_run, demcz_rhat_partial)");
    HIPCHK(h, hipSetDevice(h->cfg.device_id));
    int32_t rc = live_verify(h);
    if (rc) return rc;
    if (h->no_live && h->rearm_from >= g_from) h->rearm_from = g_from - 1;
    const bool pacing = (getenv("DEMCZ_NO_HOST_PACING") == nullptr);
    for (;;) {
        h->host_paced = pacing;
        h->in_checked = true;
        rc = run_checked_body(h, g_from, g_to, gamma, temperature, every, threshold, g_stop, n_checks, rhat_max, n_max, rhat_last);
        h->host_paced = false;
        h->in_checked = false;
        if (h->live_log.empty()) break;
        if (rc != DEMCZ_OK && h->peer_mode == 2) break;
        bool failed = false;
        { int32_t rcf = live_failed(h, failed); if (rcf) { rc = rcf; break; } }
        if (!failed) { h->live_log.clear(); break; }
        std::vector<demcz_handle::RunCall> dropped;
        rc = live_rollback(h, dropped);
        if (rc) break;
        h->replaying = true;
    }
    h->replaying = false;
    return rc;
}

extern "C" int32_t demcz_set_live_spin_limit(demcz_handle* h, int32_t polls)
{
    if (!h || polls < 0) return DEMCZ_ERR_INVALID_ARGUMENT;
    h->live_spin_limit = (unsigned int)polls;
    return DEMCZ_OK;
}

extern "C" int32_t demcz_set_live_rearms(demcz_handle* h, int32_t n)
{
    if (!h || n < 0) return DEMCZ_ERR_INVALID_ARGUMENT;
    h->live_rearms_left = n;
    if (h->peer_mode == 1 && h->group) {
        h->group->rearms_left = n;
        for (demcz_handle* m : h->group->members) m->live_rearms_left = n;
    }
    if (n == 0) h->rearm_from = -1;
    return DEMCZ_OK;
}

extern "C" int32_t demcz_get_live_rearms(const demcz_handle* h, int32_t* rearms, int32_t* left)
{
    if (!h) return DEMCZ_ERR_INVALID_ARGUMENT;
    if (rearms) *rearms = h->live_rearms;
    if (left) *left = h->live_rearms_left;
    return DEMCZ_OK;
}

extern "C" int32_t demcz_debug_set_live_fault(demcz_handle* h, int32_t polls, int64_t g_from)
{
    if (!h || polls < -1 || g_from < 0) return DEMCZ_ERR_INVALID_ARGUMENT;
    h->live_fault_polls = polls;
    h->live_fault_g = g_from;
    return DEMCZ_OK;
}

extern "C" int32_t demcz_debug_kernel_counts(const demcz_handle* h, int64_t* counts)
{
    if (!h || !counts) return DEMCZ_ERR_INVALID_ARGUMENT;
    const bool wave = h->lanes == DEMCZ_LAYOUT_SPLIT && h->split_kind == SPLIT_WAVE;
    counts[0] = h->kernel_counts[0];
    counts[1] = wave ? h->launches - h->kernel_counts[0] : 0;
    counts[2] = wave ? 0 : h->launches;
    return DEMCZ_OK;
}

extern "C" int32_t demcz_debug_kernel_name(const demcz_handle* h, char* buf, int32_t cap)
{
    if (!h || !buf || cap < 1) return DEMCZ_ERR_INVALID_ARGUMENT;
    const int d = h->cfg.d;
    const char* tg = h->cfg.target_kind == DEMCZ_TARGET_MVNORMAL ? "MVNORMAL" : h->cfg.target_kind == DEMCZ_TARGET_ISO_QUAD ? "ISO_QUAD"
                     : h->cfg.target_kind == DEMCZ_TARGET_LINREG_SSE ? "LINREG_SSE" : h->cfg.target_kind == DEMCZ_TARGET_PROGRAM ? "PROGRAM" : "HOST";
    const WindowKernel k = h->last_kernel.threads ? h->last_kernel : window_kernel_of(h, launch_facts(h, nullptr, false));
    const char* lv = k.live ? "true" : "false";
    const char* tm = k.temper ? "true" : "false";
    char tmp[160];
    switch (k.arm) {
    case ARM_LR8S: snprintf(tmp, sizeof tmp, "window_kernel_lr8s<%d, %s>", d, lv); break;
    case ARM_PROGRAM_WAVE: snprintf(tmp, sizeof tmp, "%s<%d, %d, %s, %s> (program)", d <= 5 ? "window_kernel_ps" : "window_kernel_pw", (int)TARGET_PROGRAM, d, lv, tm); break;
    case ARM_PS: snprintf(tmp, sizeof tmp, "window_kernel_ps<%s, %d, %s, %s>", tg, d, lv, tm); break;
    case ARM_PS2: snprintf(tmp, sizeof tmp, "window_kernel_ps2<%s, %d, %s, %s>", tg, d, lv, tm); break;
    case ARM_PS2D: snprintf(tmp, sizeof tmp, "window_kernel_ps2d<%s, %d, %s, %s>", tg, d, lv, tm); break;
    case ARM_PW:
        snprintf(tmp, sizeof tmp, "window_kernel_pw<%s, %d, %s, %s%s>", tg, d, lv, tm,
                 k.pw_form == PW_FORM_MATRIX ? ", true" : k.pw_form == PW_FORM_REGULAR ? ", false, true" : "");
        break;
    case ARM_MLB_REC:
        if (h->mlb_qb > 0 && h->split_lanes == 16) snprintf(tmp, sizeof tmp, "window_kernel_mlb<%s, %d, %d, true, %s, %d>", tg, d, h->split_lanes, lv, h->mlb_qb);
        else snprintf(tmp, sizeof tmp, "window_kernel_mlb<%s, %d, %d, true, %s>", tg, d, h->split_lanes, lv);
        break;
    case ARM_LR16_REC: snprintf(tmp, sizeof tmp, "window_kernel_lr16<%d, true, %s>", d, lv); break;
    case ARM_ML_REC: snprintf(tmp, sizeof tmp, "window_kernel_ml<%s, %d, 16, true, %s>", tg, d, lv); break;
    case ARM_PC8: snprintf(tmp, sizeof tmp, "window_kernel_pc8<%s, %d, %s, %s>", tg, d, lv, tm); break;
    case ARM_MLB: snprintf(tmp, sizeof tmp, "window_kernel_mlb<%s, %d, %d>", tg, d, h->lanes); break;
    case ARM_LR16: snprintf(tmp, sizeof tmp, "window_kernel_lr16<%d, false, false>", d); break;
    case ARM_ML_COOP: snprintf(tmp, sizeof tmp, "window_kernel_ml<%s, %d, %d, false, false, true>", tg, d, h->lanes); break;
    case ARM_ML: snprintf(tmp, sizeof tmp, "window_kernel_ml<%s, %d, %d>", tg, d, h->lanes); break;
    case ARM_ONE_LANE:
        if (h->cfg.target_kind == DEMCZ_TARGET_PROGRAM) snprintf(tmp, sizeof tmp, "window_kernel<%d, %d, %s> (program)", (int)TARGET_PROGRAM, d, h->full_block ? "true" : "false");
        else snprintf(tmp, sizeof tmp, "window_kernel<%s, %d, %s>", tg, d, h->full_block ? "true" : "false");
        break;
    }
    snprintf(buf, (size_t)cap, "demcz::%s", tmp);
    return DEMCZ_OK;
}

extern "C" int32_t demcz_get_live_status(const demcz_handle* h, int32_t* live_enabled, int32_t* redos)
{
    if (!h) return DEMCZ_ERR_INVALID_ARGUMENT;
    if (live_enabled) *live_enabled = (h->lanes == DEMCZ_LAYOUT_SPLIT && !h->no_live && h->live_claimed) ? 1 : 0;
    if (redos) *redos = h->live_redos;
    return DEMCZ_OK;
}

extern "C" int32_t demcz_debug_append_slab(demcz_handle* h, const double* slab, int32_t R, int32_t cnt, int32_t batched)
{
    if (!h || !slab || R < 1 || cnt < 1 || (!batched && cnt != 1)) return DEMCZ_ERR_INVALID_ARGUMENT;
    if (!h->has_state) return fail(h, DEMCZ_ERR_STATE, "demcz_debug_append_slab: no state");
    if (h->lag != 0 || !h->pending.empty()) return fail(h, DEMCZ_ERR_STATE, "demcz_debug_append_slab: rows are pending");
    const int64_t N = h->cfg.N, rows = N * R * cnt;
    const int d = h->cfg.d;
    if (h->M_app + rows > h->cfg.Mcap) return fail(h, DEMCZ_ERR_CAPACITY, "demcz_debug_append_slab: Z capacity exceeded");
    HIPCHK(h, hipSetDevice(h->cfg.device_id));
    int32_t rc = ensure_scratch(h, rows * d);
    if (rc) return rc;
    HIPCHK(h, hipMemcpyAsync(h->d_scratch, slab, (size_t)rows * d * sizeof(double), hipMemcpyHostToDevice, h->stream));
    const int64_t tot = rows * d;
    if (batched)
        hipLaunchKernelGGL(append_batch_kernel, dim3((unsigned)((tot + 255) / 256)), dim3(256), 0, h->stream, h->dZ, h->ZS,
                           h->M_app, (const double*)h->d_scratch, N, (int)R, (int)cnt, d);
    else
        hipLaunchKernelGGL(append_gathered_kernel, dim3((unsigned)((tot + 255) / 256)), dim3(256), 0, h->stream, h->dZ, h->ZS,
                           h->M_app, (const double*)h->d_scratch, N, (int)R, d);
    HIPCHK(h, hipGetLastError());
    SYNCCHK(h, h->stream);
    h->M_app += rows;
    h->M = h->M_app;
    rec_invalidate(h);
    return DEMCZ_OK;
}

extern "C" int32_t demcz_set_kernel_timing(demcz_handle* h, int32_t enabled)
{
    if (!h) return DEMCZ_ERR_INVALID_ARGUMENT;
    h->timing = enabled != 0;
    return DEMCZ_OK;
// ... 40 lines not shown
```

### demc.jl_amd/csrc/demcz_kernels.h

```cpp
#pragma once

#include "demcz_device.h"

#pragma clang fp contract(off)

#ifdef DEMCZ_STAMPS
#define DEMCZ_STAMP(P, i) do { if ((P).stamps && threadIdx.x == 0 && blockIdx.x < 65536u) (P).stamps[(size_t)blockIdx.x * 16 + (i)] = __builtin_readcyclecounter(); } while (0)
#else
#define DEMCZ_STAMP(P, i) do { } while (0)
#endif

namespace demcz {

enum { TARGET_MVNORMAL = 0, TARGET_ISO_QUAD = 1, TARGET_LINREG_SSE = 2, TARGET_HOST_CALLBACK = 3, TARGET_PROGRAM = 4 };

constexpr int MAX_D = 64;
constexpr int LINREG_PARTIALS = 16;
constexpr int WINDOW_BS = 64;

struct TargetParams {
    const double* mu;
    const double* Wp;
    double c0;
    const double* design;
    const double* yobs;
    int64_t nobs;
    int32_t ngrp;
    const int32_t* goff;
    uint64_t gstart;
};

constexpr int DEMCZ_MAX_PEERS = 7;

struct WindowParams {
    const double* Z;
    double* Zw;
    int64_t ZS;
    int64_t M;
    double* Xcur;
    double* lpcur;
    double* chain;
    double* logobj;
    const double* temperature;
    int64_t N;
    int64_t chain_id0;
    int32_t d;
    int32_t ngen;
    int64_t g_first;
    int64_t slot_first;
    double gamma;
    uint64_t seed;
    int64_t S;
    int32_t Nblocks;
    int32_t do_append;
    int64_t M_append;
    double* snap;
    int32_t K;
    int32_t to_boundary;
    const int32_t* block_offsets;
    const int32_t* slot_of;
    const double* eps;
    TargetParams tp;
    const double* rec_in;
    double* rec_out;
    int64_t rec_stride;
    int32_t rec_fields;
    const int32_t* slot_role;
    int64_t next_g_first;
    int64_t next_M;
    int64_t next_rows;
    int32_t next_boff;
    int32_t next_ngen;
    int32_t consumer_blocks;
    unsigned int* live_err;
    int32_t live_spin_limit;
    unsigned int* acc_out;
    double* safe_X;
    double* safe_lp;
    int64_t brows;
    int64_t row_off;
    int32_t n_peers;
    double* peer_Z[DEMCZ_MAX_PEERS];
    uint32_t z_bytes;
    uint32_t hist_bytes;
#ifdef DEMCZ_STAMPS
    unsigned long long* stamps;
#endif
};

constexpr int DEMCZ_XCDS = 8;
__device__ __forceinline__ int xcd_block(int nblocks)
{
    const int b = (int)blockIdx.x;
    if (b >= nblocks || nblocks % DEMCZ_XCDS != 0) return b;
    return (b % DEMCZ_XCDS) * (nblocks / DEMCZ_XCDS) + b / DEMCZ_XCDS;
}
__device__ __forceinline__ int xcd_block(const WindowParams& P) { return xcd_block(P.consumer_blocks > 0 ? (int)P.consumer_blocks : (int)gridDim.x); }

__device__ __forceinline__ unsigned int wave_count_changed(double lp_after, double lp_before, unsigned long long speak64)
{
    const double df = lp_after - lp_before;
    const unsigned long long m = __builtin_amdgcn_fcmp(df, 0.0, 14 );
    return (unsigned int)__builtin_popcountll(m & speak64);
}
__device__ __forceinline__ void wave_store_counts(const WindowParams& P, int64_t wave, unsigned int total, unsigned int first)
{
    if (P.acc_out && (threadIdx.x & 63) == 0) {
        P.acc_out[2 * wave] = total;
        P.acc_out[2 * wave + 1] = first;
    }
}

template <int D>
__device__ __forceinline__ void load_row(const double* __restrict__ row, double (&v)[D])
{
    const double2* r2 = reinterpret_cast<const double2*>(row);
#pragma unroll
    for (int k = 0; k < D / 2; ++k) {
        double2 t = r2[k];
        v[2 * k] = t.x;
        v[2 * k + 1] = t.y;
    }
    if constexpr (D & 1) v[D - 1] = row[D - 1];
}

template <int D>
__device__ __forceinline__ void store_row(double* __restrict__ row, const double (&v)[D])
{
    double2* r2 = reinterpret_cast<double2*>(row);
#pragma unroll
    for (int k = 0; k < D / 2; ++k) r2[k] = make_double2(v[2 * k], v[2 * k + 1]);
    if constexpr (D & 1) row[D - 1] = v[D - 1];
}

template <int TARGET, int D, class XF>
__device__ __forceinline__ double target_logp(const TargetParams& tp, int d, XF X)
{
    const int dd = (D > 0) ? D : d;
    if constexpr (TARGET == TARGET_MVNORMAL) {
        if (tp.ngrp > 1) {
            if constexpr (D > 0) {
                double q = 0.0, Qg = 0.0;
                bool haveq = false;
#pragma unroll
                for (int i = 0; i < D; ++i) {
                    const double* wrow = tp.Wp + (i * (i + 1)) / 2;
                    double y = 0.0, acc = 0.0;
                    bool have = false;
#pragma unroll
                    for (int j = 0; j <= i; ++j) {
                        const bool st = (tp.gstart >> j) & 1ull;
                        const double rr = X(j) - tp.mu[j];
                        const double ysum = have ? y + acc : acc;
                        if (st && j > 0) { y = ysum; have = true; }
                        const double prod = wrow[j] * rr, fm = fma(wrow[j], rr, acc);
                        acc = st ? prod : fm;
                    }
                    y = have ? y + acc : acc;
                    const bool sti = (tp.gstart >> i) & 1ull;
                    const double qsum = haveq ? q + Qg : Qg;
                    if (sti && i > 0) { q = qsum; haveq = true; }
                    const double sq = y * y, fq = fma(y, y, Qg);
                    Qg = sti ? sq : fq;
                }
                q = haveq ? q + Qg : Qg;
                return fma(-0.5, q, tp.c0);
            } else {
// ... 260 lines not shown
    rng_state st;
    rng_seek(st, P.seed, (uint64_t)(P.chain_id0 + c), (uint64_t)(P.g_first - 1) * (uint64_t)P.S);
    int to_b = P.to_boundary;
    int64_t nb = 0;
    unsigned int cnt_total = 0, cnt_first = 0;
    const unsigned long long speak64 = __builtin_amdgcn_ballot_w64(true);

    for (int gi = 0; gi < P.ngen; ++gi) {
        const double lp_gen0 = lp;
        for (int ib = 0; ib < P.Nblocks; ++ib) {
            uint64_t r1, r2, i1, i2;
            rng_next(st, r1, r2);
            draw_rows(r1, r2, (uint64_t)P.M, i1, i2);
            const int b = P.block_offsets[ib + 1] - P.block_offsets[ib];
            const int nn = (b == 1) ? 1 : b;
            const int npairs = (nn + 1) / 2;
            for (int pr = 0; pr < npairs; ++pr) {
                rng_next(st, r1, r2);
                double z0, z1;
                normal_pair(r1, r2, z0, z1);
                zs[(2 * pr) * WINDOW_BS + tid] = z0;
                zs[(2 * pr + 1) * WINDOW_BS + tid] = z1;
            }
            const double scale = (b == 1) ? P.gamma : P.gamma / sqrt((double)(2 * b));
            const int32_t* so = P.slot_of + ib * d;
            const double* za = P.Z + (int64_t)i1 * P.ZS;
            const double* zb = P.Z + (int64_t)i2 * P.ZS;
            for (int p = 0; p < d; ++p) {
                const int t = so[p];
                double xv = xs[p * WINDOW_BS + tid];
                if (t >= 0) {
                    double diff = za[p] - zb[p];
                    double zt = zs[((b == 1) ? 0 : t) * WINDOW_BS + tid];
                    double t1 = scale * diff;
                    double t2 = P.eps[p] * zt;
                    double delta = t1 + t2;
                    xv = xv + delta;
                }
                xps[p * WINDOW_BS + tid] = xv;
            }
            rng_next(st, r1, r2);
            const double logu = dm_log(u_open(r1));
            const double lpp = target_logp<TARGET, 0>(P.tp, d, [&](int j) { return xps[j * WINDOW_BS + tid]; });
            double dlt = lpp - lp;
            if (P.temperature) dlt = dlt / P.temperature[gi];
            if (logu < dlt) {
                for (int p = 0; p < d; ++p) xs[p * WINDOW_BS + tid] = xps[p * WINDOW_BS + tid];
                lp = lpp;
            }
        }
        {
            const unsigned int k = wave_count_changed(lp, lp_gen0, speak64);
            cnt_total += k;
            cnt_first = (gi == 0) ? k : cnt_first;
        }
        const int64_t slot = P.slot_first + gi;
        if (P.chain) {
            for (int p = 0; p < d; ++p) P.chain[c + P.N * (p + (int64_t)d * slot)] = xs[p * WINDOW_BS + tid];
            P.logobj[c + P.N * slot] = lp;
        }
        if (--to_b == 0) {
            to_b = P.K;
            for (int p = 0; p < d; ++p) {
                const double xv = xs[p * WINDOW_BS + tid];
                if (P.do_append) P.Zw[(P.M_append + nb * P.N + c) * P.ZS + p] = xv;
                if (P.snap) P.snap[nb * P.N * d + c + P.N * p] = xv;
            }
            ++nb;
        }
    }
    for (int p = 0; p < d; ++p) P.Xcur[c + P.N * p] = xs[p * WINDOW_BS + tid];
    P.lpcur[c] = lp;
    wave_store_counts(P, blockIdx.x, cnt_total, cnt_first);
}

template <int TARGET>
__global__ void logp_kernel(TargetParams tp, int d, const double* X, int64_t ldX, int64_t n, double* out)
{
    const int64_t c = (int64_t)blockIdx.x * blockDim.x + threadIdx.x;
    if (c >= n) return;
    out[c] = target_logp<TARGET, 0>(tp, d, [&](int j) { return X[c + ldX * j]; });
}

#ifndef DEMCZ_NO_AUX_KERNELS
__global__ void fill_u64_kernel(unsigned long long* p, size_t n, unsigned long long v)
{
    const size_t i = (size_t)blockIdx.x * blockDim.x + threadIdx.x;
    if (i < n) p[i] = v;
}

__global__ void append_rows_kernel(double* Z, int64_t ZS, int64_t M, const double* rows, int64_t nrows,
                                   int64_t ldrows, int d)
{
    const int64_t i = (int64_t)blockIdx.x * blockDim.x + threadIdx.x;
    if (i >= nrows * d) return;
    const int64_t r = i % nrows, p = i / nrows;
    Z[(M + r) * ZS + p] = rows[r + ldrows * p];
}

__global__ void export_rows_kernel(const double* Z, int64_t ZS, int64_t r0, double* out, int64_t nrows, int64_t ldout, int d)
{
    const int64_t i = (int64_t)blockIdx.x * blockDim.x + threadIdx.x;
    if (i >= nrows * d) return;
    const int64_t r = i % nrows, p = i / nrows;
    out[r + ldout * p] = Z[(r0 + r) * ZS + p];
}

__global__ void append_gathered_kernel(double* Z, int64_t ZS, int64_t M, const double* slab, int64_t n_loc,
                                       int R, int d)
{
    const int64_t i = (int64_t)blockIdx.x * blockDim.x + threadIdx.x;
    const int64_t per = n_loc * d;
    if (i >= per * R) return;
    const int64_t r = i / per, rem = i % per, p = rem / n_loc, j = rem % n_loc;
    Z[(M + r * n_loc + j) * ZS + p] = slab[i];
}

__global__ void append_batch_kernel(double* Z, int64_t ZS, int64_t base, const double* slab, int64_t n_loc, int R, int cnt, int d)
{
    const int64_t i = (int64_t)blockIdx.x * blockDim.x + threadIdx.x;
    const int64_t per = n_loc * d;
    if (i >= per * cnt * R) return;
    const int64_t r = i / (per * cnt), rem = i % (per * cnt), sidx = rem / per, rem2 = rem % per, p = rem2 / n_loc, j = rem2 % n_loc;
    Z[(base + (sidx * R + r) * n_loc + j) * ZS + p] = slab[i];
}

__global__ void rhat_moments_kernel(const double* chain, int64_t N, int d, int64_t s0, int64_t n, int nchunk,
                                    double* S1, double* S2)
{
    const int64_t i = (int64_t)blockIdx.x * blockDim.x + threadIdx.x;
    if (i >= N * d) return;
    const int h = blockIdx.y / nchunk, ck = blockIdx.y % nchunk;
    const int64_t per = (n + nchunk - 1) / nchunk;
    const int64_t t0 = ck * per, t1 = (t0 + per < n) ? t0 + per : n;
    const int64_t stride = N * d;
    const double* base = chain + i + stride * (s0 + h * n);
    const double x0 = base[0];
    double a = 0.0, b = 0.0;
    int64_t t = t0;
    for (; t + 8 <= t1; t += 8) {
        double v[8];
#pragma unroll
        for (int u = 0; u < 8; ++u) v[u] = base[stride * (t + u)];
#pragma unroll
        for (int u = 0; u < 8; ++u) {
            const double w = v[u] - x0;
            a += w;
            b = fma(w, w, b);
        }
    }
    for (; t < t1; ++t) {
        double v = base[stride * t] - x0;
        a += v;
        b = fma(v, v, b);
    }
    const int64_t o = i + stride * blockIdx.y;
    S1[o] = a;
    S2[o] = b;
}

__global__ void rhat_chainstats_kernel(const double* chain, int64_t N, int d, int64_t s0, int64_t n, int nchunk,
                                       const double* S1, const double* S2, double* mean_j, double* s2_j)
{
    const int64_t i = (int64_t)blockIdx.x * blockDim.x + threadIdx.x;
    if (i >= N * d) return;
    const int h = blockIdx.y;
    const int64_t stride = N * d;
    const double x0 = chain[i + stride * (s0 + h * n)];
    double a = 0.0, b = 0.0;
    for (int ck = 0; ck < nchunk; ++ck) {
        a += S1[i + stride * (h * nchunk + ck)];
        b += S2[i + stride * (h * nchunk + ck)];
    }
    const double nn = (double)n;
    mean_j[i + stride * h] = x0 + a / nn;
    s2_j[i + stride * h] = (b - a * a / nn) / (nn - 1.0);
}

__global__ void __launch_bounds__(256) rhat_reduce_kernel(const double* mean_j, const double* s2_j, int64_t N, int d,
                                                          int stage, const double* grand, double grand_div, double* out)
{
    __shared__ double ra[256], rb[256];
    const int p = blockIdx.x;
    const int64_t stride = N * d;
    double a = 0.0, b = 0.0;
    const double gm = stage ? grand[p] / grand_div : 0.0;
    int64_t h = 0, c = threadIdx.x;
    while (c >= N) { c -= N; ++h; }
    for (int64_t k = threadIdx.x; k < 2 * N; k += 256) {
        const int64_t at = c + N * p + stride * h;
        const double mj = mean_j[at];
        if (stage == 0) {
            a += mj;
        } else {
            const double dv = mj - gm;
            a = fma(dv, dv, a);
            b += s2_j[at];
        }
        c += 256;
        while (c >= N) { c -= N; ++h; }
    }
    ra[threadIdx.x] = a;
    rb[threadIdx.x] = b;
    __syncthreads();
    for (int s = 128; s > 0; s >>= 1) {
        if ((int)threadIdx.x < s) {
            ra[threadIdx.x] += ra[threadIdx.x + s];
            rb[threadIdx.x] += rb[threadIdx.x + s];
        }
        __syncthreads();
    }
    if (threadIdx.x == 0) {
        out[p] = ra[0];
        if (stage) out[d + p] = rb[0];
    }
}

__global__ void __launch_bounds__(256) rhat_tail_kernel(const double* mean_j, const double* s2_j, int64_t N, int d,
                                                        double n, double m, double* rhat)
{
    __shared__ double ra[256], rb[256];
    const int p = blockIdx.x;
    const int64_t stride = N * d;
    double a = 0.0, b = 0.0;
    int64_t h0 = 0, c0 = threadIdx.x;
    while (c0 >= N) { c0 -= N; ++h0; }
    {
        int64_t h = h0, c = c0;
        for (int64_t k = threadIdx.x; k < 2 * N; k += 256) {
            a += mean_j[c + N * p + stride * h];
            c += 256;
            while (c >= N) { c -= N; ++h; }
        }
    }
    ra[threadIdx.x] = a;
    __syncthreads();
    for (int s = 128; s > 0; s >>= 1) {
        if ((int)threadIdx.x < s) ra[threadIdx.x] += ra[threadIdx.x + s];
        __syncthreads();
    }
    const double gm = ra[0] / m;
    __syncthreads();
    a = 0.0;
    {
        int64_t h = h0, c = c0;
        for (int64_t k = threadIdx.x; k < 2 * N; k += 256) {
            const int64_t at = c + N * p + stride * h;
            const double dv = mean_j[at] - gm;
            a = fma(dv, dv, a);
            b += s2_j[at];
            c += 256;
            while (c >= N) { c -= N; ++h; }
        }
    }
    ra[threadIdx.x] = a;
    rb[threadIdx.x] = b;
    __syncthreads();
    for (int s = 128; s > 0; s >>= 1) {
        if ((int)threadIdx.x < s) {
            ra[threadIdx.x] += ra[threadIdx.x + s];
            rb[threadIdx.x] += rb[threadIdx.x + s];
        }
        __syncthreads();
    }
    if (threadIdx.x == 0) {
        const double B = n / (m - 1.0) * ra[0];
        const double W = rb[0] / m;
        const double varhat = (n - 1.0) / n * W + B / n;
        rhat[p] = sqrt(varhat / W);
    }
}

__global__ void rhat_final_kernel(const double* in, int d, double n, double m, double* rhat)
{
    const int p = blockIdx.x * blockDim.x + threadIdx.x;
    if (p >= d) return;
    const double B = n / (m - 1.0) * in[p];
    const double W = in[d + p] / m;
    const double varhat = (n - 1.0) / n * W + B / n;
    rhat[p] = sqrt(varhat / W);
}

__global__ void __launch_bounds__(256) changed_from_history_kernel(const double* logobj, const double* lp_origin, int64_t N,
                                                                   int64_t s_from, long long* out)
{
    __shared__ int cnt[256];
    const int64_t s = s_from + blockIdx.x;
    const double* cur = logobj + N * s;
    const double* prev = (s == 0) ? lp_origin : logobj + N * (s - 1);
    int k = 0;
    for (int64_t c = threadIdx.x; c < N; c += 256) k += ((cur[c] - prev[c]) != 0.0) ? 1 : 0;
    cnt[threadIdx.x] = k;
    __syncthreads();
    for (int st = 128; st > 0; st >>= 1) {
        if ((int)threadIdx.x < st) cnt[threadIdx.x] += cnt[threadIdx.x + st];
        __syncthreads();
    }
    if (threadIdx.x == 0) out[blockIdx.x] = cnt[0];
}

__global__ void __launch_bounds__(64) changed_per_chain_kernel(const double* logobj, int64_t N, int64_t s0, int64_t w, int nchunk,
                                                               unsigned int* cnt)
{
    const int64_t c = (int64_t)blockIdx.x * 64 + threadIdx.x;
    if (c >= N) return;
    const int64_t per = (w - 1 + nchunk - 1) / nchunk;
    const int64_t t0 = 1 + (int64_t)blockIdx.y * per, t1 = (t0 + per < w) ? t0 + per : w;
    if (t0 >= t1) return;
    unsigned int k = 0;
    double prev = logobj[c + N * (s0 + t0 - 1)];
    for (int64_t t = t0; t < t1; ++t) {
        const double cur = logobj[c + N * (s0 + t)];
        k += ((cur - prev) != 0.0) ? 1u : 0u;
        prev = cur;
    }
    atomicAdd(&cnt[c], k);
}

__global__ void changed_ratio_kernel(const unsigned int* cnt, int64_t N, int64_t w, double* ratio)
{
    const int64_t c = (int64_t)blockIdx.x * blockDim.x + threadIdx.x;
    if (c < N) ratio[c] = (double)cnt[c] / (double)(w - 1);
}

constexpr int MC_TS = 8;
constexpr int MC_VALS = MC_TS * MC_TS + MC_TS;

__global__ void __launch_bounds__(256) meancov_partial_kernel(const double* chain, int64_t N, int d, int64_t s0, int64_t w, int nchunk,
                                                              double* partial)
{
    __shared__ double red[4][MC_VALS];
    const int T = (d + MC_TS - 1) / MC_TS;
    int I = 0, J = (int)blockIdx.z;
    while (J >= T - I) { J -= T - I; ++I; }
    J += I;
    const int64_t c = (int64_t)blockIdx.x * 256 + threadIdx.x;
    const int64_t per = (w + nchunk - 1) / nchunk;
    const int64_t t0 = (int64_t)blockIdx.y * per, t1 = (t0 + per < w) ? t0 + per : w;
    const int64_t stride = N * d;
    double acc[MC_TS][MC_TS], sm[MC_TS];
#pragma unroll
    for (int a = 0; a < MC_TS; ++a) {
        sm[a] = 0.0;
#pragma unroll
        for (int b = 0; b < MC_TS; ++b) acc[a][b] = 0.0;
    }
    if (c < N) {
        double ri[MC_TS], rj[MC_TS];
#pragma unroll
        for (int a = 0; a < MC_TS; ++a) {
            ri[a] = (I * MC_TS + a < d) ? chain[N * (I * MC_TS + a) + stride * s0] : 0.0;
            rj[a] = (J * MC_TS + a < d) ? chain[N * (J * MC_TS + a) + stride * s0] : 0.0;
        }
// ... 77 lines not shown
```

### demc.jl_amd/csrc/demcz_kernels_ps.h

```cpp
#pragma once

#include "demcz_kernels_pc.h"

#pragma clang fp contract(off)

namespace demcz {

constexpr int PS_CHAINS = 4;
constexpr int PS_R = 5;
constexpr int PS_PUB = 4;
#ifndef PS_AHEAD_N
#define PS_AHEAD_N 2
#endif
constexpr int PS_AHEAD = PS_AHEAD_N;
constexpr int PS_SLOTS = PS_AHEAD + 1;
constexpr int PS_MAX_N = 2048;

__device__ __forceinline__ void ps_dma16(const void* gsrc, unsigned lds_dst)
{
    unsigned keep;
    asm volatile("s_mov_b32 %0, m0\n\ts_mov_b32 m0, %2\n\ts_nop 0\n\tglobal_load_lds_dwordx4 %1, off\n\ts_mov_b32 m0, %0"
                 : "=&s"(keep) : "v"(gsrc), "s"(lds_dst) : "memory");
}

constexpr int PRODUCE_WAVES = 4;
constexpr size_t PRODUCE_THROTTLE_LDS = 64 * 1024;
template <int D>
__global__ void __launch_bounds__(64 * PRODUCE_WAVES) produce_kernel(const WindowParams P)
{
    pc_produce<D>(P, (int64_t)blockIdx.x * PRODUCE_WAVES + (int64_t)(threadIdx.x >> 6), (int)(threadIdx.x & 63));
}

template <int TARGET, int D, bool LIVE, bool TEMPER>
__global__ void __launch_bounds__(64 * (PS_CHAINS + (LIVE ? 1 : 0)), 3) window_kernel_ps(const WindowParams P)
{
#ifdef DEMCZ_PROGRAM_TARGET
    static_assert(TARGET == TARGET_MVNORMAL || TARGET == TARGET_ISO_QUAD || TARGET == TARGET_PROGRAM, "split layout: MvNormal / isotropic / program targets");
#else
    static_assert(TARGET == TARGET_MVNORMAL || TARGET == TARGET_ISO_QUAD, "split layout: MvNormal / isotropic targets");
#endif
    static_assert(D >= 2 && D <= 5, "a pass's rows, normals, log u and indices are one 64-lane DMA");
    constexpr bool PROG = (TARGET == TARGET_PROGRAM);
    constexpr int HW = (D + 1) / 2;
    constexpr int ZSC = (D <= 2) ? 2 : (D <= 4) ? 4 : 8;
    constexpr int ZSH = (ZSC == 2) ? 4 : (ZSC == 4) ? 5 : 6;
    constexpr int DP = ((D + 1) / 2) * 2;
    constexpr int CR = ((D + 2) / 2) * 2;
    constexpr int ROWL = PS_R * 2 * HW;
    constexpr int FL0 = ROWL;
    constexpr int TL0 = FL0 + 3 * (D + 2);
    static_assert(TL0 + 3 <= 64, "one DMA instruction per pass");
    const int lane = threadIdx.x & 63;
    const int w = __builtin_amdgcn_readfirstlane((int)(threadIdx.x >> 6));
    if constexpr (!LIVE) {
        if ((int64_t)blockIdx.x >= P.consumer_blocks) {
            pc_produce<D>(P, ((int64_t)blockIdx.x - P.consumer_blocks) * PS_CHAINS + w, lane);
            return;
        }
    }
    __shared__ __attribute__((aligned(16))) unsigned char raw[PS_CHAINS][PS_SLOTS][1024];
    __shared__ __attribute__((aligned(16))) double sdelta[PS_CHAINS][(PS_R + 1) * DP];
    __shared__ __attribute__((aligned(16))) double ctab[PS_CHAINS][2][32 * CR];
    __shared__ double pub_rows[LIVE ? PS_CHAINS * PS_PUB * D : 1];
    __shared__ unsigned int pub_seq[PS_CHAINS], pub_done[PS_CHAINS], pub_exit[PS_CHAINS];
    if constexpr (LIVE) {
        if (threadIdx.x < PS_CHAINS) { pub_seq[threadIdx.x] = 0u; pub_done[threadIdx.x] = 0u; pub_exit[threadIdx.x] = 0u; }
        __syncthreads();
        if (w == PS_CHAINS) {
            const bool pl = lane < PS_CHAINS * D;
            const int cw = pl ? lane / D : 0, pp = pl ? lane % D : 0;
            const int64_t cl = (int64_t)xcd_block(P) * PS_CHAINS + cw;
            unsigned int done = 0u;
            while (true) {
                publisher_wait(P);
                const unsigned int seq = __hip_atomic_load(&pub_seq[cw], __ATOMIC_RELAXED, __HIP_MEMORY_SCOPE_WORKGROUP);
                const bool ready = pl && seq != done;
                if (__builtin_amdgcn_ballot_w64(ready) != 0ull) {
                    if (ready) {
                        const double v = pub_rows[(cw * PS_PUB + (int)(done % PS_PUB)) * D + pp];
                        if (cl < P.N && P.do_append) live_publish(P, (int64_t)done, cl, pp, v);
                        ++done;
                    }
                    asm volatile("" ::: "memory");
                    if (ready && pp == 0) __hip_atomic_store(&pub_done[cw], done, __ATOMIC_RELAXED, __HIP_MEMORY_SCOPE_WORKGROUP);
                    continue;
                }
                const bool gone = !pl || (__hip_atomic_load(&pub_exit[cw], __ATOMIC_RELAXED, __HIP_MEMORY_SCOPE_WORKGROUP) != 0u &&
                                          __hip_atomic_load(&pub_seq[cw], __ATOMIC_RELAXED, __HIP_MEMORY_SCOPE_WORKGROUP) == done);
                if (__builtin_amdgcn_ballot_w64(!gone) == 0ull) break;
                __builtin_amdgcn_s_sleep(1);
            }
            return;
        }
    }
    auto leave = [&]() {
        asm volatile("s_waitcnt vmcnt(0)" ::: "memory");
        if constexpr (LIVE) {
            if (lane == 0) __hip_atomic_store(&pub_exit[w], 1u, __ATOMIC_RELAXED, __HIP_MEMORY_SCOPE_WORKGROUP);
        }
    };
    const int64_t c = (int64_t)xcd_block(P) * PS_CHAINS + w;
    if (c >= P.N) {
        wave_store_counts(P, c, 0u, 0u);
        leave();
        return;
    }
    if constexpr (LIVE) {
        if (__hip_atomic_load(P.live_err, __ATOMIC_RELAXED, __HIP_MEMORY_SCOPE_AGENT) != 0u) { leave(); return; }
    }
    __builtin_amdgcn_s_setprio(3);
    unsigned char* const raw_w = &raw[w][0][0];
    double* const sd_w = &sdelta[w][0];
    double* const ct_w = &ctab[w][0][0];
// ... 410 lines not shown
```

### demc.jl_amd/csrc/demcz_kernels_rec.h

```cpp
#pragma once

#include "demcz_kernels.h"

#pragma clang fp contract(off)

namespace demcz {

struct philox_blocks : rocrand_device::philox4x32_10_engine {
    __device__ __forceinline__ philox_blocks() {}
    __device__ __forceinline__ void block(uint64_t seed, uint64_t chain, uint64_t blk, uint64_t& r1, uint64_t& r2)
    {
        uint4 ctr = {(unsigned)blk, (unsigned)(blk >> 32), (unsigned)chain, (unsigned)(chain >> 32)};
        uint2 key = {(unsigned)seed, (unsigned)(seed >> 32)};
        uint4 w = this->ten_rounds(ctr, key);
        r1 = (uint64_t)w.x | ((uint64_t)w.y << 32);
        r2 = (uint64_t)w.z | ((uint64_t)w.w << 32);
    }
};

__device__ __forceinline__ void wave_lds_handoff()
{
    asm volatile("" ::: "memory");
    __builtin_amdgcn_wave_barrier();
    asm volatile("" ::: "memory");
}

__device__ __forceinline__ size_t rec_index(int64_t N, int64_t GS, int g, int f, int64_t c) { return ((size_t)f * (size_t)N + (size_t)c) * (size_t)GS + (size_t)g; }
__device__ __forceinline__ size_t rec_index_rm(int64_t N, int F, int g, int f, int64_t c) { return ((size_t)g * (size_t)N + (size_t)c) * (size_t)F + (size_t)f; }

__host__ __device__ inline bool produce_by_generation(int32_t rec_fields, int32_t ngen) { return rec_fields == 0 && ngen >= 64; }
__host__ __device__ inline int64_t produce_units(int64_t N, int roles, int32_t rec_fields, int32_t ngen)
{
    return produce_by_generation(rec_fields, ngen) ? N * roles * (int64_t)((ngen + 63) / 64) : ((N + 63) / 64) * roles * (int64_t)ngen;
}

template <int D>
__device__ __forceinline__ void pc_produce(const WindowParams& P, int64_t pb, int lane = -1)
{
    if (lane < 0) lane = (int)threadIdx.x;
    constexpr int NPAIRS = (D == 1) ? 1 : (D + 1) / 2;
    constexpr int S = NPAIRS + 2;
    int64_t c;
    int role, gi;
    if (produce_by_generation(P.rec_fields, P.next_ngen)) {
        const int64_t gblocks = (P.next_ngen + 63) / 64;
        const int64_t per_chain = (int64_t)S * gblocks;
        c = pb / per_chain;
        const int64_t rem = pb % per_chain;
        role = (int)(rem / gblocks);
        gi = (int)(rem % gblocks) * 64 + lane;
    } else {
        const int64_t nbc = (P.N + 63) / 64;
        const int64_t plane = pb / nbc;
        c = (pb % nbc) * 64 + lane;
        role = (int)(plane % S);
        gi = (int)(plane / S);
    }
    if (gi >= P.next_ngen || c >= P.N) return;
    philox_blocks rng;
    uint64_t r1, r2;
    rng.block(P.seed, (uint64_t)(P.chain_id0 + c), (uint64_t)(P.next_g_first + gi - 1) * (uint64_t)S + (uint64_t)role, r1, r2);
    double* rec = P.rec_out;
    auto at = [&](int g, int f) -> size_t {
        return P.rec_fields ? rec_index_rm(P.N, P.rec_fields, g, f, c) : rec_index(P.N, P.rec_stride, g, f, c);
    };
    if (role == 0) {
        const int64_t Mg = P.next_M + (int64_t)((gi + P.next_boff) / P.K) * P.next_rows;
        uint64_t i1, i2;
        draw_rows(r1, r2, (uint64_t)Mg, i1, i2);
        rec[at(gi, D + 1)] = __longlong_as_double((long long)(i1 | (i2 << 32)));
    } else {
        const double lg = dm_log(u_open(r1));
        if (role == S - 1) {
            rec[at(gi, D)] = lg;
        } else {
            const double R = sqrt(-2.0 * lg);
            double cs, sn;
            dm_sincos2pi(r2 >> 11, cs, sn);
            const int p0 = (D == 1) ? 0 : 2 * (role - 1);
            rec[at(gi, p0)] = R * cs;
            if (p0 + 1 < D) rec[at(gi, p0 + 1)] = R * sn;
        }
    }
}

__device__ __forceinline__ void pcb_produce(const WindowParams& P, int64_t pb)
{
    const int64_t nbc = (P.N + 63) / 64;
    const int64_t plane = pb / nbc;
    const int64_t c = (pb % nbc) * 64 + (threadIdx.x & 63);
    const int s = (int)(plane % P.S), gi = (int)(plane / P.S);
    if (gi >= P.next_ngen || c >= P.N) return;
    const int role = P.slot_role[s];
    philox_blocks rng;
    uint64_t r1, r2;
    rng.block(P.seed, (uint64_t)(P.chain_id0 + c), (uint64_t)(P.next_g_first + gi - 1) * (uint64_t)P.S + (uint64_t)s, r1, r2);
    double2 e;
    if (role == 0) {
        const int64_t Mg = P.next_M + (int64_t)((gi + P.next_boff) / P.K) * P.next_rows;
        uint64_t i1, i2;
        draw_rows(r1, r2, (uint64_t)Mg, i1, i2);
        e.x = __longlong_as_double((long long)i1);
        e.y = __longlong_as_double((long long)i2);
    } else {
        const double lg = dm_log(u_open(r1));
        if (role == 2) {
            e.x = lg;
            e.y = 0.0;
        } else {
            const double R = sqrt(-2.0 * lg);
            double cs, sn;
            dm_sincos2pi(r2 >> 11, cs, sn);
            e.x = R * cs;
            e.y = R * sn;
        }
    }
    reinterpret_cast<double2*>(P.rec_out)[((size_t)gi * (size_t)P.N + (size_t)c) * (size_t)P.S + (size_t)s] = e;
}

constexpr unsigned long long LIVE_SENTINEL = 0xFFF4DEADC0DE5EEDull;
constexpr int LIVE_SPIN_LIMIT = 1 << 18;

__device__ __forceinline__ double live_load(const double* p)
{
    return __hip_atomic_load(p, __ATOMIC_RELAXED, __HIP_MEMORY_SCOPE_AGENT);
}
__device__ __forceinline__ void live_store(double* p, double v)
{
    __hip_atomic_store(p, v, __ATOMIC_RELAXED, __HIP_MEMORY_SCOPE_AGENT);
}
__device__ __forceinline__ bool is_sentinel(double v) { return (unsigned long long)__double_as_longlong(v) == LIVE_SENTINEL; }
__device__ __forceinline__ unsigned long long sentinel_lanes(double v)
{
    return __builtin_amdgcn_uicmpl((unsigned long long)__double_as_longlong(v), LIVE_SENTINEL, 32 );
}

__device__ __forceinline__ void live_store_sys(double* p, double v)
{
    __hip_atomic_store(p, v, __ATOMIC_RELAXED, __HIP_MEMORY_SCOPE_SYSTEM);
}
__device__ __forceinline__ void live_publish(const WindowParams& P, int64_t b, int64_t cl, int p, double v)
{
    const int64_t off = (P.M_append + b * P.brows + P.row_off + cl) * P.ZS + p;
    live_store(P.Zw + off, v);
    for (int r = 0; r < P.n_peers; ++r) live_store_sys(P.peer_Z[r] + off, v);
}
__device__ __forceinline__ void publisher_wait(const WindowParams&)
{
#ifdef DEMCZ_PUB_WAIT
    asm volatile("s_waitcnt vmcnt(0)" ::: "memory");
#else
    asm volatile("s_waitcnt vmcnt(40)" ::: "memory");
#endif
}
__device__ __forceinline__ double live_reload(const WindowParams& P, const double* p)
{
    if (P.n_peers > 0) return __hip_atomic_load(p, __ATOMIC_RELAXED, __HIP_MEMORY_SCOPE_SYSTEM);
    return live_load(p);
}


__device__ __forceinline__ bool live_poll_abandon(const WindowParams& P, int& spins, bool lane_waiting, unsigned row, int gi)
{
    const bool timeout = (++spins >= P.live_spin_limit);
// ... 13 lines not shown
```

### demc.jl_amd/engine.py

```python
from __future__ import annotations

import ctypes as C

import numpy as np

from . import _lib
from ._lib import DemczError
from .targets import is_device_target


def blocks_to_csr(blockindex, d):
    blocks = [np.asarray(list(b), dtype=np.int64) for b in blockindex]
    for b in blocks:
        if b.size == 0 or b.min() < 0 or b.max() >= d:
            raise ValueError("block indices must be 0-based and within [0, d)")
    offs = np.zeros(len(blocks) + 1, dtype=np.int32)
    offs[1:] = np.cumsum([b.size for b in blocks])
    idx = np.concatenate(blocks).astype(np.int32)
    return offs, idx


class _PinnedOwner:

    def __init__(self, L, bases):
# ... 51 lines not shown

    def _chk(self, rc):
        if rc != 0:
            raise DemczError(rc, (self._L.demcz_last_error(self._h) or b"").decode())

    def close(self):
        if getattr(self, "_h", None) is not None and self._h.value:
            self._L.demcz_destroy(self._h)
            self._h = C.c_void_p()

    def __del__(self):
        try:
            self.close()
        except Exception:
            pass

    def set_state(self, X, logp, Z):
        X = _lib.f64(X, "F")
        Z = _lib.f64(Z, "F")
        if X.shape != (self.N, self.d) or Z.ndim != 2 or Z.shape[1] != self.d:
            raise ValueError("X must be N x d and Z must be M0 x d")
        lp = _lib.f64(logp) if logp is not None else None
        if lp is not None and lp.shape != (self.N,):
            raise ValueError("logp must have N entries")
        self._chk(self._L.demcz_set_state(self._h, _lib.ptr(X), _lib.ptr(lp), _lib.ptr(Z), Z.shape[0], Z.shape[0]))

    def get_state(self, with_Z=True):
        X = np.empty((self.N, self.d), order="F")
        lp = np.empty(self.N)
        M = C.c_int64()
        self._chk(self._L.demcz_get_state(self._h, _lib.ptr(X), _lib.ptr(lp), None, 0, C.byref(M)))
        Z = None
        if with_Z:
            pz, Mz = C.c_void_p(), C.c_int64()
            self._chk(self._L.demcz_get_archive_pinned(self._h, C.byref(pz), C.byref(Mz)))
            buf = (C.c_double * (Mz.value * self.d)).from_address(pz.value)
            buf._owner = _PinnedOwner(self._L, [pz.value])
            Z = np.ctypeslib.as_array(buf).reshape((Mz.value, self.d), order="F")
        return X, lp, Z, int(M.value)

    @property
    def M(self):
        M = C.c_int64()
        self._chk(self._L.demcz_get_info(self._h, C.byref(M), None, None))
        return int(M.value)

    def info(self):
        M, nl, lanes = C.c_int64(), C.c_int64(), C.c_int32()
        self._chk(self._L.demcz_get_info(self._h, C.byref(M), C.byref(nl), C.byref(lanes)))
        return dict(M=int(M.value), window_launches=int(nl.value), lanes_per_chain=int(lanes.value))

    def set_append_lag(self, batches):
        self._chk(self._L.demcz_set_append_lag(self._h, int(batches)))

    def set_rng_offset(self, generations):
        self._chk(self._L.demcz_set_rng_offset(self._h, int(generations)))

    def set_history_origin(self, g0):
        self._chk(self._L.demcz_set_history_origin(self._h, int(g0)))

    def run(self, g_from, g_to, gamma, temperature=None):
        t = None
        if temperature is not None:
            t = _lib.f64(temperature)
            if t.shape != (g_to - g_from + 1,):
                raise ValueError("one temperature per generation")
        self._chk(self._L.demcz_run(self._h, int(g_from), int(g_to), float(gamma), _lib.ptr(t)))

    def run_checked(self, g_from, g_to, gamma, every, threshold=0.0, temperature=None):
        t = None
        if temperature is not None:
            t = _lib.f64(temperature)
            if t.shape != (g_to - g_from + 1,):
                raise ValueError("one temperature per generation")
        n_max = int((g_to - g_from + 1) // every + 2)
        mx = np.zeros(n_max)
        last = np.full(self.d, np.nan)
        g_stop, n = C.c_int64(0), C.c_int32(0)
        self._chk(self._L.demcz_run_checked(self._h, C.c_int64(int(g_from)), C.c_int64(int(g_to)), C.c_double(float(gamma)),
                                            _lib.ptr(t), C.c_int64(int(every)), C.c_double(float(threshold)), C.byref(g_stop),
                                            C.byref(n), _lib.ptr(mx), C.c_int32(n_max), _lib.ptr(last)))
        return int(g_stop.value), mx[:n.value].copy(), last

    def set_kernel_timing(self, enabled: bool):
        self._chk(self._L.demcz_set_kernel_timing(self._h, C.c_int32(1 if enabled else 0)))

    def get_kernel_time(self):
        n, ms = C.c_int64(0), C.c_double(0.0)
        self._chk(self._L.demcz_get_kernel_time(self._h, C.byref(n), C.byref(ms)))
        return int(n.value), float(ms.value)

    def get_kernel_time_series(self):
        n = C.c_int32(0)
        self._chk(self._L.demcz_get_kernel_time_series(self._h, 0, None, None, C.byref(n)))
        st, du = np.zeros(n.value), np.zeros(n.value)
        self._chk(self._L.demcz_get_kernel_time_series(self._h, n.value, _lib.ptr(st), _lib.ptr(du), C.byref(n)))
        return st, du

    def set_live_spin_limit(self, polls: int):
        self._chk(self._L.demcz_set_live_spin_limit(self._h, C.c_int32(int(polls))))

    def debug_set_live_fault(self, polls: int, g_from: int = 0):
        self._chk(self._L.demcz_debug_set_live_fault(self._h, C.c_int32(int(polls)), C.c_int64(int(g_from))))

    def live_status(self):
        on, redos = C.c_int32(0), C.c_int32(0)
        self._chk(self._L.demcz_get_live_status(self._h, C.byref(on), C.byref(redos)))
        return bool(on.value), int(redos.value)

    def set_live_rearms(self, n: int):
        self._chk(self._L.demcz_set_live_rearms(self._h, C.c_int32(int(n))))

    def live_rearms(self):
        a, b = C.c_int32(0), C.c_int32(0)
        self._chk(self._L.demcz_get_live_rearms(self._h, C.byref(a), C.byref(b)))
        return int(a.value), int(b.value)

    def kernel_counts(self):
        c = (C.c_int64 * 3)()
        self._chk(self._L.demcz_debug_kernel_counts(self._h, c))
        return dict(zip(("ps2", "ps_general", "other"), (int(v) for v in c)))

    def kernel_name(self):
        buf = C.create_string_buffer(192)
        self._chk(self._L.demcz_debug_kernel_name(self._h, buf, 192))
        return buf.value.decode()

    def synchronize(self):
        self._chk(self._L.demcz_synchronize(self._h))

    def get_history(self, g_from, g_to, chain=True, log_obj=True, out=None):
        G = g_to - g_from + 1
        if out is not None and chain and log_obj:
            ch_full, lo_full = out
            ok = (ch_full.flags.f_contiguous and lo_full.flags.f_contiguous and ch_full.shape[:2] == (self.N, self.d)
                  and lo_full.shape[0] == self.N and ch_full.shape[2] >= G and lo_full.shape[1] >= G
                  and ch_full.dtype == np.float64 and lo_full.dtype == np.float64)
            if ok:
                self._chk(self._L.demcz_get_history(self._h, int(g_from), int(g_to), _lib.ptr(ch_full), _lib.ptr(lo_full)))
                return ch_full[:, :, :G], lo_full[:, :G]
        ch = np.empty((self.N, self.d, G), order="F") if chain else None
        lo = np.empty((self.N, G), order="F") if log_obj else None
        self._chk(self._L.demcz_get_history(self._h, int(g_from), int(g_to), _lib.ptr(ch), _lib.ptr(lo)))
        return ch, lo

    def history_stream(self, enabled=True):
        self._chk(self._L.demcz_history_stream(self._h, 1 if enabled else 0))
        self._streaming = bool(enabled)

    def take_history(self, g_from, g_to):
        G = g_to - g_from + 1
        pc, pl = C.c_void_p(), C.c_void_p()
        self._chk(self._L.demcz_get_history_view(self._h, int(g_from), int(g_to), C.byref(pc), C.byref(pl)))
        bc, bl = C.c_void_p(), C.c_void_p()
        self._chk(self._L.demcz_detach_history(self._h, C.byref(bc), C.byref(bl)))
        self._streaming = False
        owner = _PinnedOwner(self._L, [bc.value, bl.value])
        cbuf = (C.c_double * (self.N * self.d * G)).from_address(pc.value)
        lbuf = (C.c_double * (self.N * G)).from_address(pl.value)
        cbuf._owner = owner
        lbuf._owner = owner
        chain = np.ctypeslib.as_array(cbuf).reshape((self.N, self.d, G), order="F")
        lobj = np.ctypeslib.as_array(lbuf).reshape((self.N, G), order="F")
        return chain, lobj

    def get_changed(self, g_from, g_to):
        out = np.zeros(g_to - g_from + 1, dtype=np.int64)
        self._chk(self._L.demcz_get_changed(self._h, int(g_from), int(g_to), _lib.ptr(out, _lib._lp)))
        return out

    def changed_total(self, g_from, g_to, with_source=False):
        tot, src = C.c_int64(0), C.c_int32(0)
        self._chk(self._L.demcz_get_changed_total(self._h, int(g_from), int(g_to), C.byref(tot), C.byref(src)))
        return (int(tot.value), bool(src.value)) if with_source else int(tot.value)

    def rhat(self, g_from, g_to):
        out = np.empty(self.d)
        self._chk(self._L.demcz_rhat(self._h, int(g_from), int(g_to), _lib.ptr(out)))
        return out

    def rhat_partial(self, g_from, g_to, stage, grand):
        out = np.empty(self.d if stage == 0 else 2 * self.d)
        g = _lib.f64(grand) if grand is not None else None
        self._chk(self._L.demcz_rhat_partial(self._h, int(g_from), int(g_to), int(stage), _lib.ptr(g), _lib.ptr(out)))
        return out

    def accept_ratio(self, g_from, g_to):
        out = np.empty(self.N)
        self._chk(self._L.demcz_accept_ratio(self._h, int(g_from), int(g_to), _lib.ptr(out)))
        return out

    def mean_cov(self, g_from, g_to):
        mean = np.empty(self.d)
        cov = np.empty((self.d, self.d), order="F")
        self._chk(self._L.demcz_mean_cov(self._h, int(g_from), int(g_to), _lib.ptr(mean), _lib.ptr(cov)))
        return mean, cov

    def closure_buffers(self):
        if getattr(self, "_hc", None) is None:
            px, pl = C.c_void_p(), C.c_void_p()
            self._chk(self._L.demcz_closure_buffers(self._h, C.byref(px), C.byref(pl)))
            bx = (C.c_double * (self.N * self.d)).from_address(px.value)
            bl = (C.c_double * self.N).from_address(pl.value)
            self._hc = (np.ctypeslib.as_array(bx).reshape((self.N, self.d), order="F"), np.ctypeslib.as_array(bl))
# ... 114 lines not shown
```

### include/demcz.h

```cpp
#ifndef DEMCZ_H
#define DEMCZ_H

#include <stdint.h>

#ifdef __cplusplus
extern "C" {
#endif

typedef struct demcz_handle demcz_handle;

enum demcz_status {
    DEMCZ_OK = 0,
    DEMCZ_ERR_INVALID_ARGUMENT = 1,
    DEMCZ_ERR_HIP = 2,
    DEMCZ_ERR_CAPACITY = 3,
    DEMCZ_ERR_STATE = 4,
    DEMCZ_ERR_NO_DEVICE = 5,
    DEMCZ_ERR_COMM = 6
};

enum demcz_target_kind {
    DEMCZ_TARGET_MVNORMAL = 0,
    DEMCZ_TARGET_ISO_QUAD = 1,
    DEMCZ_TARGET_LINREG_SSE = 2,
// ... 32 lines not shown

int32_t demcz_program_check(int32_t d, const char* source, const char* options);
int32_t demcz_program_check_layout(int32_t d, const char* source, const char* options, int32_t lanes_per_chain);
int32_t demcz_set_program(demcz_handle* h, const char* source, const char* options, const double* data, int64_t ndata);

#define DEMCZ_ABI_VERSION 1
int32_t demcz_abi_version(void);

int32_t demcz_create(demcz_handle** out, const demcz_config* cfg);
int32_t demcz_destroy(demcz_handle* h);
const char* demcz_last_error(const demcz_handle* h);

int32_t demcz_set_state(demcz_handle* h, const double* X, const double* logp,
                        const double* Z, int64_t ldZ, int64_t M0);

int32_t demcz_get_state(demcz_handle* h, double* X, double* logp, double* Z, int64_t ldZ, int64_t* M);

int32_t demcz_get_archive_pinned(demcz_handle* h, double** Z, int64_t* M);

int32_t demcz_set_history_origin(demcz_handle* h, int64_t g0);

int32_t demcz_run(demcz_handle* h, int64_t g_from, int64_t g_to, double gamma, const double* temperature);

int32_t demcz_synchronize(demcz_handle* h);

int32_t demcz_get_history(demcz_handle* h, int64_t g_from, int64_t g_to, double* chain, double* log_obj);

int32_t demcz_history_stream(demcz_handle* h, int32_t enabled);
int32_t demcz_get_history_view(demcz_handle* h, int64_t g_from, int64_t g_to, double** chain, double** log_obj);
int32_t demcz_detach_history(demcz_handle* h, void** chain_base, void** logobj_base);
int32_t demcz_release_host_buffer(void* base);

int32_t demcz_pool_trim(int64_t* device_bytes_freed, int64_t* pinned_bytes_freed);

int32_t demcz_get_changed(demcz_handle* h, int64_t g_from, int64_t g_to, int64_t* changed);

int32_t demcz_get_changed_total(demcz_handle* h, int64_t g_from, int64_t g_to, int64_t* total, int32_t* from_ballots);

int32_t demcz_rhat(demcz_handle* h, int64_t g_from, int64_t g_to, double* rhat);

int32_t demcz_rhat_partial(demcz_handle* h, int64_t g_from, int64_t g_to, int32_t stage,
                           const double* grand, double* out);

int32_t demcz_accept_ratio(demcz_handle* h, int64_t g_from, int64_t g_to, double* ratio);

int32_t demcz_mean_cov(demcz_handle* h, int64_t g_from, int64_t g_to, double* mean, double* cov);

int32_t demcz_propose(demcz_handle* h, int64_t g, int32_t ib, double gamma, double* Xprop);
int32_t demcz_closure_buffers(demcz_handle* h, double** Xprop, double** logp);
int32_t demcz_accept_commit(demcz_handle* h, const double* logp_prop, const double* temperature);
int32_t demcz_end_generation(demcz_handle* h, int64_t g);

int32_t demcz_comm_unique_id(void* unique_id_128B);
int32_t demcz_comm_init(demcz_handle* h, const void* unique_id_128B, int32_t nranks, int32_t rank);

int32_t demcz_peer_group(demcz_handle** handles, int32_t R);
int32_t demcz_get_peer_status(const demcz_handle* h, int32_t* mode, int32_t* peers);
int32_t demcz_peer_export(demcz_handle* h, int32_t nranks, int32_t rank, void* handle_64B);
int32_t demcz_peer_attach(demcz_handle* h, const void* handles_64B_each);
int32_t demcz_peer_detach(demcz_handle* h);
int32_t demcz_get_peer_ping(const demcz_handle* h, int32_t* ok, double* wait_us);

int32_t demcz_set_comm_timeout(demcz_handle* h, int64_t milliseconds);

int32_t demcz_export_current_device(demcz_handle* h, double* X_device);
int32_t demcz_append_rows_device(demcz_handle* h, const double* rows_device, int64_t nrows, int64_t ldrows);
int32_t demcz_append_rows(demcz_handle* h, const double* rows, int64_t nrows, int64_t ldrows);
int32_t demcz_set_external_append(demcz_handle* h, int32_t enabled);

int32_t demcz_set_append_lag(demcz_handle* h, int32_t batches);

int32_t demcz_set_rng_offset(demcz_handle* h, int64_t generations);

int32_t demcz_rhat_array(int32_t device_id, const double* chain, int64_t N, int32_t d, int64_t G, double* rhat);
int32_t demcz_accept_ratio_array(int32_t device_id, const double* log_obj, int64_t N, int64_t G, double* ratio);
int32_t demcz_mean_cov_array(int32_t device_id, const double* chain, int64_t N, int32_t d, int64_t G, double* mean, double* cov);

int32_t demcz_get_info(const demcz_handle* h, int64_t* M, int64_t* launches_window, int32_t* lanes_per_chain);

int32_t demcz_run_checked(demcz_handle* h, int64_t g_from, int64_t g_to, double gamma, const double* temperature,
                          int64_t every, double threshold, int64_t* g_stop, int32_t* n_checks,
                          double* rhat_max, int32_t n_max, double* rhat_last);


int32_t demcz_set_kernel_timing(demcz_handle* h, int32_t enabled);
int32_t demcz_get_kernel_time(demcz_handle* h, int64_t* launches, double* milliseconds);

int32_t demcz_get_kernel_time_series(demcz_handle* h, int32_t cap, double* start_ms, double* duration_ms, int32_t* n);

int32_t demcz_selftest_draws(int32_t device_id, uint64_t seed, uint64_t chain, uint64_t blk0, int32_t n,
                             uint64_t* words, double* normals, double* logu);

int32_t demcz_set_live_spin_limit(demcz_handle* h, int32_t polls);
int32_t demcz_get_live_status(const demcz_handle* h, int32_t* live_enabled, int32_t* redos);
int32_t demcz_set_live_rearms(demcz_handle* h, int32_t n);
int32_t demcz_get_live_rearms(const demcz_handle* h, int32_t* rearms, int32_t* left);
int32_t demcz_debug_kernel_counts(const demcz_handle* h, int64_t* counts);
int32_t demcz_debug_kernel_name(const demcz_handle* h, char* buf, int32_t cap);

int32_t demcz_debug_set_live_fault(demcz_handle* h, int32_t polls, int64_t g_from);

int32_t demcz_debug_stall_exchange(demcz_handle* h, int32_t milliseconds);

int32_t demcz_debug_append_slab(demcz_handle* h, const double* slab, int32_t R, int32_t cnt, int32_t batched);

#ifdef __cplusplus
}
#endif
#endif
```

Before: 689.3 million.

## Fuse parked R-hat moment computation into the producer kernel launch

Instead of launching standalone R-hat moment and chainstat kernels on the side stream during checked runs, the check is parked and its moment work is folded into the next producer kernel's blocks. A single finish kernel that recomputes chain stats in LDS then writes R-hat, directly to mapped host memory when it can. The aim is to cut kernel launches and side-stream contention during convergence checks. The producer kernel also gains a waves-per-EU hint, and extra branches in the producer may add register pressure.

```diff
diff --git a/demc.jl_amd/_lib.py b/demc.jl_amd/_lib.py
--- a/demc.jl_amd/_lib.py
+++ b/demc.jl_amd/_lib.py
@@ -38,7 +38,7 @@
     "demcz_debug_kernel_counts", "demcz_pool_trim", "demcz_debug_kernel_name", "demcz_peer_group", "demcz_get_peer_status", "demcz_peer_export", "demcz_peer_attach",
     "demcz_peer_detach", "demcz_get_peer_ping", "demcz_set_live_rearms", "demcz_get_live_rearms",
     "demcz_closure_buffers", "demcz_program_check", "demcz_set_program",
-    "demcz_program_check_layout",
+    "demcz_program_check_layout", "demcz_get_checked_rhat", "demcz_debug_check_counts",
 ]
 
 
@@ -154,6 +154,8 @@
     L.demcz_set_live_spin_limit.argtypes = [C.c_void_p, C.c_int32]
     L.demcz_get_live_status.argtypes = [C.c_void_p, _ip, _ip]
     L.demcz_debug_kernel_counts.argtypes = [C.c_void_p, _lp]
+    L.demcz_debug_check_counts.argtypes = [C.c_void_p, _lp]
+    L.demcz_get_checked_rhat.argtypes = [C.c_void_p, C.c_int32, _dp]
     L.demcz_history_stream.argtypes = [C.c_void_p, C.c_int32]
     L.demcz_get_history_view.argtypes = [C.c_void_p, C.c_int64, C.c_int64, C.POINTER(C.c_void_p), C.POINTER(C.c_void_p)]
     L.demcz_detach_history.argtypes = [C.c_void_p, C.POINTER(C.c_void_p), C.POINTER(C.c_void_p)]
diff --git a/demc.jl_amd/csrc/demcz_capi.hip b/demc.jl_amd/csrc/demcz_capi.hip
--- a/demc.jl_amd/csrc/demcz_capi.hip
+++ b/demc.jl_amd/csrc/demcz_capi.hip
@@ -229,6 +229,9 @@
     hipEvent_t diag_ev = nullptr;
     hipEvent_t rhat_side_ev = nullptr;
     bool rhat_side_pending = false;
+    struct { bool active = false; int64_t g_from = 0, g_to = 0; double* out = nullptr; } rhat_parked;
+    int64_t checks_fused = 0, checks_standalone = 0;
+    int32_t last_checks = 0;
     double* d_spec_X = nullptr;
     double* d_spec_lp = nullptr;
     hipEvent_t spec_ev = nullptr;
@@ -1068,6 +1071,7 @@
     if (!X || !Z) return fail(h, DEMCZ_ERR_INVALID_ARGUMENT, "demcz_set_state: X and Z are required");
     if (M0 < 2) return fail(h, DEMCZ_ERR_INVALID_ARGUMENT, "demcz_set_state: M0 >= 2 needed (two distinct archive rows, demcz.jl:176-179)");
     if (M0 > h->cfg.Mcap || ldZ < M0) return fail(h, DEMCZ_ERR_CAPACITY, "demcz_set_state: M0 exceeds Mcap or ldZ < M0");
+    h->rhat_parked.active = false;
     if (!logp && h->cfg.target_kind == DEMCZ_TARGET_HOST_CALLBACK)
         return fail(h, DEMCZ_ERR_INVALID_ARGUMENT, "demcz_set_state: host-callback target needs logp");
     if (h->cfg.target_kind == DEMCZ_TARGET_PROGRAM && !h->prog_ready)
@@ -1345,6 +1349,10 @@
     return live && !no_reg && P.K % PS_R == 0 && P.to_boundary % PS_R == 0 && P.ngen % PS_R == 0 && P.ngen >= PS_R;
 }
 
+static int32_t rhat_flush_parked(demcz_handle* h);
+static int32_t rhat_take_parked(demcz_handle* h, WindowParams& P, int64_t units, bool& taken);
+static int32_t rhat_finish_parked(demcz_handle* h, const WindowParams& P, hipStream_t qs);
+
 static int32_t launch_window_pc(demcz_handle* h, const WindowParams& P, const WindowKernel& k, bool live = false)
 {
     const int64_t nbc = (P.N + 63) / 64;
@@ -1357,13 +1365,26 @@
         if (h->split_kind == SPLIT_WAVE && P.ZS != ((P.d <= 2) ? 2 : (P.d <= 4) ? 4 : ((P.d + 7) / 8) * 8)) return fail(h, DEMCZ_ERR_STATE, "split layout: archive row stride");
         const int bin = (P.rec_in == h->d_rec[0]) ? 0 : 1, bout = (P.rec_out == h->d_rec[0]) ? 0 : 1;
         const bool one_launch = !live && P.consumer_blocks > 0;
+        static const bool serial_env = getenv("DEMCZ_PRODUCE_SERIAL") != nullptr;
+        WindowParams PF;
+        const WindowParams* PP = &P;
+        bool fused = false;
+        if (h->rhat_parked.active && P.consumer_blocks > 0) {
+            if (units > 0 && live && !serial_env && h->peer_mode == 0 && !h->comm && h->split_kind == SPLIT_WAVE && !h->lr_spec && !h->ps_dual &&
+                !h->replaying && pc_records && produce_by_generation(P.rec_fields, P.next_ngen)) {
+                PF = P;
+                int32_t rcp = rhat_take_parked(h, PF, units, fused);
+                if (rcp) return rcp;
+                if (fused) PP = &PF;
+            }
+            if (!fused) { int32_t rcp = rhat_flush_parked(h); if (rcp) return rcp; }
+        }
         if (units > 0 && one_launch && h->prod_pending[bout]) {
             HIPCHK(h, hipStreamWaitEvent(h->stream, h->prod_done[bout], 0));
             h->prod_pending[bout] = false;
         }
         if (units > 0 && !one_launch) {
             hipStream_t ps = h->stream;
-            static const bool serial_env = getenv("DEMCZ_PRODUCE_SERIAL") != nullptr;
             if (P.consumer_blocks > 0 && !serial_env && h->peer_mode != 1) {
                 if (!h->prod_stream) {
                     HIPCHK(h, stream_acquire(h->cfg.device_id, &h->prod_stream));
@@ -1401,7 +1422,7 @@
             }
             const size_t dyn = (ps != h->stream) ? (h->lr_spec ? (size_t)8192 : (h->ps_dual && !getenv("DEMCZ_PRODUCE_LDS")) ? (size_t)32768 : big_d) : 0;
             switch (P.d) {
-#define DEMCZ_PRODUCE_CASE(DD) case DD: hipLaunchKernelGGL((produce_kernel<DD>), pg, pw, dyn, ps, P); break;
+#define DEMCZ_PRODUCE_CASE(DD) case DD: hipLaunchKernelGGL((produce_kernel<DD>), pg, pw, dyn, ps, *PP); break;
             DEMCZ_PRODUCE_CASE(2) DEMCZ_PRODUCE_CASE(3) DEMCZ_PRODUCE_CASE(4) DEMCZ_PRODUCE_CASE(5) DEMCZ_PRODUCE_CASE(6) DEMCZ_PRODUCE_CASE(7)
             DEMCZ_PRODUCE_CASE(8) DEMCZ_PRODUCE_CASE(9) DEMCZ_PRODUCE_CASE(10) DEMCZ_PRODUCE_CASE(11) DEMCZ_PRODUCE_CASE(12) DEMCZ_PRODUCE_CASE(13)
             DEMCZ_PRODUCE_CASE(14) DEMCZ_PRODUCE_CASE(15) DEMCZ_PRODUCE_CASE(16) DEMCZ_PRODUCE_CASE(17) DEMCZ_PRODUCE_CASE(18) DEMCZ_PRODUCE_CASE(19)
@@ -1415,6 +1436,11 @@
             if (ps != h->stream) {
                 HIPCHK(h, hipEventRecord(h->prod_done[bout], ps));
                 h->prod_pending[bout] = true;
+            }
+            if (fused) {
+                if (ps != h->prod_stream) return fail(h, DEMCZ_ERR_STATE, "launch_window_pc: a fused check without the producer stream");
+                int32_t rcf = rhat_finish_parked(h, *PP, ps);
+                if (rcf) return rcf;
             }
         }
         if (P.consumer_blocks > 0) {
@@ -1863,6 +1889,7 @@
 {
     calls.swap(h->live_log);
     h->live_log.clear();
+    h->rhat_parked.active = false;
     const int64_t N = h->cfg.N;
     const int d = h->cfg.d;
     SYNCCHK(h, h->stream);
@@ -2351,6 +2378,7 @@
     P.safe_X = nullptr; P.safe_lp = nullptr;
     P.rec_in = nullptr; P.rec_out = nullptr; P.next_g_first = 0; P.next_M = 0; P.next_ngen = 0; P.consumer_blocks = 0;
     P.next_rows = 0; P.next_boff = 0; P.rec_stride = 0;
+    P.mom_hist = nullptr; P.mom_s0 = 0; P.mom_n = 0; P.mom_S1 = nullptr; P.mom_S2 = nullptr; P.mom_stride = 0; P.mom_nchunk = 0; P.mom_tasks = 0;
     P.rec_fields = (h->lanes == DEMCZ_LAYOUT_SPLIT && h->split_kind == SPLIT_ML) ? h->cfg.d + 2 : 0;
     P.z_bytes = (uint32_t)std::min<size_t>(h->dZ_bytes, 0xffffffffull);
     P.hist_bytes = (hist && h->hist_joint) ? (uint32_t)std::min<double>((double)h->cfg.N * (h->cfg.d + 1) * (double)h->cfg.Gcap * 8.0, 4294967295.0) : 0u;
@@ -2725,12 +2753,20 @@
     return DEMCZ_OK;
 }
 
-static int32_t rhat_enqueue(demcz_handle* h, int64_t g_from, int64_t g_to, double* out, bool side = false)
+static int32_t rhat_enqueue(demcz_handle* h, int64_t g_from, int64_t g_to, double* out, bool side = false, bool may_park = true)
 {
     RhatPlan r;
     hipStream_t qs = h->stream;
+    if (h->rhat_parked.active) { int32_t rcp = rhat_flush_parked(h); if (rcp) return rcp; }
     static const bool own_env = getenv("DEMCZ_RHAT_OWN_STREAM") != nullptr;
     if (side && !h->comm && !own_env && h->prod_stream) {
+        static const bool no_fused = getenv("DEMCZ_NO_FUSED_CHECK") != nullptr && atoi(getenv("DEMCZ_NO_FUSED_CHECK")) != 0;
+        if (may_park && !no_fused && h->in_checked && h->peer_mode == 0 && h->split_kind == SPLIT_WAVE && !h->ps_dual) {
+            int32_t rcp = rhat_prepare(h, g_from, g_to, r, false);
+            if (rcp) return rcp;
+            h->rhat_parked.active = true; h->rhat_parked.g_from = g_from; h->rhat_parked.g_to = g_to; h->rhat_parked.out = out;
+            return DEMCZ_OK;
+        }
         if (!h->diag_ev) HIPCHK(h, hipEventCreateWithFlags(&h->diag_ev, hipEventDisableTiming));
         if (h->after_launch_ev) {
             HIPCHK(h, hipStreamWaitEvent(h->prod_stream, h->after_launch_ev, 0));
@@ -2776,6 +2812,7 @@
     } side_mark{h, qs};
     int32_t rc = rhat_prepare(h, g_from, g_to, r, true, qs);
     if (rc) return rc;
+    ++h->checks_standalone;
     const int d = r.d;
     const int64_t n = r.n;
     const int64_t m = 2 * r.N * h->nranks;
@@ -2797,6 +2834,52 @@
     hipLaunchKernelGGL(rhat_final_kernel, dim3((unsigned)((d + 63) / 64)), dim3(64), 0, qs, (const double*)(sums + d), d, (double)n, (double)m, sums + 3 * d);
     HIPCHK(h, hipGetLastError());
     HIPCHK(h, hipMemcpyAsync(out, sums + 3 * d, (size_t)d * sizeof(double), hipMemcpyDeviceToHost, qs));
+    return DEMCZ_OK;
+}
+
+static int32_t rhat_flush_parked(demcz_handle* h)
+{
+    if (!h->rhat_parked.active) return DEMCZ_OK;
+    h->rhat_parked.active = false;
+    return rhat_enqueue(h, h->rhat_parked.g_from, h->rhat_parked.g_to, h->rhat_parked.out, true, false);
+}
+
+static size_t rhat_finish_lds(int64_t N) { return (size_t)4 * (size_t)N * sizeof(double); }
+
+static int32_t rhat_take_parked(demcz_handle* h, WindowParams& P, int64_t units, bool& taken)
+{
+    taken = false;
+    RhatPlan r;
+    int32_t rc = rhat_prepare(h, h->rhat_parked.g_from, h->rhat_parked.g_to, r, false);
+    if (rc) return rc;
+    const int64_t tasks = ((r.nd + 63) / 64) * 2 * r.nchunk;
+    if (units < tasks || tasks > INT32_MAX || rhat_finish_lds(r.N) + 2 * 256 * sizeof(double) > 64 * 1024 || r.N != P.N || r.d != P.d) return DEMCZ_OK;
+    P.mom_hist = h->dchain; P.mom_s0 = r.s0; P.mom_n = r.n; P.mom_S1 = r.S1; P.mom_S2 = r.S2;
+    P.mom_stride = units / tasks; P.mom_nchunk = r.nchunk; P.mom_tasks = (int32_t)tasks;
+    taken = true;
+    return DEMCZ_OK;
+}
+
+static int32_t rhat_finish_parked(demcz_handle* h, const WindowParams& P, hipStream_t qs)
+{
+    h->rhat_parked.active = false;
+    RhatPlan r;
+    int32_t rc = rhat_prepare(h, h->rhat_parked.g_from, h->rhat_parked.g_to, r, false);
+    if (rc) return rc;
+    if (r.S1 != P.mom_S1) return fail(h, DEMCZ_ERR_STATE, "rhat_finish_parked: the scratch buffer moved under a fused check");
+    double* out = h->rhat_parked.out;
+    double* dev_out = nullptr;
+    if (hipHostGetDevicePointer((void**)&dev_out, out, 0) != hipSuccess) { dev_out = nullptr; (void)hipGetLastError(); }
+    double* dst = dev_out ? dev_out : r.sums + 3 * r.d;
+    const double m = (double)(2 * r.N);
+    hipLaunchKernelGGL(rhat_finish_kernel, dim3(r.d), dim3(256), rhat_finish_lds(r.N), qs, (const double*)h->dchain, r.N, r.d, r.s0, r.n, r.nchunk,
+                       (const double*)r.S1, (const double*)r.S2, m, dst);
+    HIPCHK(h, hipGetLastError());
+    if (!dev_out) HIPCHK(h, hipMemcpyAsync(out, dst, (size_t)r.d * sizeof(double), hipMemcpyDeviceToHost, qs));
+    if (!h->rhat_side_ev) HIPCHK(h, hipEventCreateWithFlags(&h->rhat_side_ev, hipEventDisableTiming));
+    HIPCHK(h, hipEventRecord(h->rhat_side_ev, qs));
+    h->rhat_side_pending = true;
+    ++h->checks_fused;
     return DEMCZ_OK;
 }
 
@@ -3722,6 +3805,9 @@
         }
         g = nxt + 1;
     }
+    if (rc == DEMCZ_OK) rc = rhat_flush_parked(h);
+    h->rhat_parked.active = false;
+    h->last_checks = 0;
     h->pinned_err_launches = -1;
     if (rc == DEMCZ_OK && !h->live_log.empty() && h->peer_mode != 2) {
         if (!h->pinned_err && host_malloc((void**)&h->pinned_err, 4 * sizeof(unsigned int)) != hipSuccess) { h->pinned_err = nullptr; (void)hipGetLastError(); }
@@ -3737,6 +3823,7 @@
             if (rhat_max && i < n_max) rhat_max[i] = max_of(pinned + (size_t)i * d);
         if (rhat_last && checks > 0) std::copy(pinned + (size_t)(checks - 1) * d, pinned + (size_t)checks * d, rhat_last);
         if (n_checks) *n_checks = checks;
+        h->last_checks = checks;
     }
     return rc;
 }
@@ -3817,6 +3904,23 @@
     counts[0] = h->kernel_counts[0];
     counts[1] = wave ? h->launches - h->kernel_counts[0] : 0;
     counts[2] = wave ? 0 : h->launches;
+    return DEMCZ_OK;
+}
+
+extern "C" int32_t demcz_debug_check_counts(const demcz_handle* h, int64_t* counts)
+{
+    if (!h || !counts) return DEMCZ_ERR_INVALID_ARGUMENT;
+    counts[0] = h->checks_fused;
+    counts[1] = h->checks_standalone;
+    return DEMCZ_OK;
+}
+
+extern "C" int32_t demcz_get_checked_rhat(demcz_handle* h, int32_t i, double* rhat)
+{
+    if (!h || !rhat) return DEMCZ_ERR_INVALID_ARGUMENT;
+    if (i < 0 || i >= h->last_checks || !h->pinned_rhat)
+        return fail(h, DEMCZ_ERR_INVALID_ARGUMENT, "demcz_get_checked_rhat: no such check in the last demcz_run_checked");
+    std::copy(h->pinned_rhat + (size_t)i * h->cfg.d, h->pinned_rhat + (size_t)(i + 1) * h->cfg.d, rhat);
     return DEMCZ_OK;
 }
 
diff --git a/demc.jl_amd/csrc/demcz_kernels.h b/demc.jl_amd/csrc/demcz_kernels.h
--- a/demc.jl_amd/csrc/demcz_kernels.h
+++ b/demc.jl_amd/csrc/demcz_kernels.h
@@ -83,6 +83,14 @@
     double* peer_Z[DEMCZ_MAX_PEERS];
     uint32_t z_bytes;
     uint32_t hist_bytes;
+    const double* mom_hist;
+    int64_t mom_s0;
+    int64_t mom_n;
+    double* mom_S1;
+    double* mom_S2;
+    int64_t mom_stride;
+    int32_t mom_nchunk;
+    int32_t mom_tasks;
 #ifdef DEMCZ_STAMPS
     unsigned long long* stamps;
 #endif
@@ -509,58 +517,12 @@
     out[c] = target_logp<TARGET, 0>(tp, d, [&](int j) { return X[c + ldX * j]; });
 }
 
-#ifndef DEMCZ_NO_AUX_KERNELS
-__global__ void fill_u64_kernel(unsigned long long* p, size_t n, unsigned long long v)
-{
-    const size_t i = (size_t)blockIdx.x * blockDim.x + threadIdx.x;
-    if (i < n) p[i] = v;
-}
-
-__global__ void append_rows_kernel(double* Z, int64_t ZS, int64_t M, const double* rows, int64_t nrows,
-                                   int64_t ldrows, int d)
-{
-    const int64_t i = (int64_t)blockIdx.x * blockDim.x + threadIdx.x;
-    if (i >= nrows * d) return;
-    const int64_t r = i % nrows, p = i / nrows;
-    Z[(M + r) * ZS + p] = rows[r + ldrows * p];
-}
-
-__global__ void export_rows_kernel(const double* Z, int64_t ZS, int64_t r0, double* out, int64_t nrows, int64_t ldout, int d)
-{
-    const int64_t i = (int64_t)blockIdx.x * blockDim.x + threadIdx.x;
-    if (i >= nrows * d) return;
-    const int64_t r = i % nrows, p = i / nrows;
-    out[r + ldout * p] = Z[(r0 + r) * ZS + p];
-}
-
-__global__ void append_gathered_kernel(double* Z, int64_t ZS, int64_t M, const double* slab, int64_t n_loc,
-                                       int R, int d)
-{
-    const int64_t i = (int64_t)blockIdx.x * blockDim.x + threadIdx.x;
-    const int64_t per = n_loc * d;
-    if (i >= per * R) return;
-    const int64_t r = i / per, rem = i % per, p = rem / n_loc, j = rem % n_loc;
-    Z[(M + r * n_loc + j) * ZS + p] = slab[i];
-}
-
-__global__ void append_batch_kernel(double* Z, int64_t ZS, int64_t base, const double* slab, int64_t n_loc, int R, int cnt, int d)
-{
-    const int64_t i = (int64_t)blockIdx.x * blockDim.x + threadIdx.x;
-    const int64_t per = n_loc * d;
-    if (i >= per * cnt * R) return;
-    const int64_t r = i / (per * cnt), rem = i % (per * cnt), sidx = rem / per, rem2 = rem % per, p = rem2 / n_loc, j = rem2 % n_loc;
-    Z[(base + (sidx * R + r) * n_loc + j) * ZS + p] = slab[i];
-}
-
-__global__ void rhat_moments_kernel(const double* chain, int64_t N, int d, int64_t s0, int64_t n, int nchunk,
-                                    double* S1, double* S2)
-{
-    const int64_t i = (int64_t)blockIdx.x * blockDim.x + threadIdx.x;
-    if (i >= N * d) return;
-    const int h = blockIdx.y / nchunk, ck = blockIdx.y % nchunk;
+__device__ __forceinline__ void rhat_moments_chunk(const double* chain, int64_t stride, int64_t i, int y, int64_t s0, int64_t n,
+                                                   int nchunk, double* S1, double* S2)
+{
+    const int h = y / nchunk, ck = y % nchunk;
     const int64_t per = (n + nchunk - 1) / nchunk;
     const int64_t t0 = ck * per, t1 = (t0 + per < n) ? t0 + per : n;
-    const int64_t stride = N * d;
     const double* base = chain + i + stride * (s0 + h * n);
     const double x0 = base[0];
     double a = 0.0, b = 0.0;
@@ -581,18 +543,65 @@
         a += v;
         b = fma(v, v, b);
     }
-    const int64_t o = i + stride * blockIdx.y;
+    const int64_t o = i + stride * y;
     S1[o] = a;
     S2[o] = b;
 }
 
-__global__ void rhat_chainstats_kernel(const double* chain, int64_t N, int d, int64_t s0, int64_t n, int nchunk,
-                                       const double* S1, const double* S2, double* mean_j, double* s2_j)
+#ifndef DEMCZ_NO_AUX_KERNELS
+__global__ void fill_u64_kernel(unsigned long long* p, size_t n, unsigned long long v)
+{
+    const size_t i = (size_t)blockIdx.x * blockDim.x + threadIdx.x;
+    if (i < n) p[i] = v;
+}
+
+__global__ void append_rows_kernel(double* Z, int64_t ZS, int64_t M, const double* rows, int64_t nrows,
+                                   int64_t ldrows, int d)
+{
+    const int64_t i = (int64_t)blockIdx.x * blockDim.x + threadIdx.x;
+    if (i >= nrows * d) return;
+    const int64_t r = i % nrows, p = i / nrows;
+    Z[(M + r) * ZS + p] = rows[r + ldrows * p];
+}
+
+__global__ void export_rows_kernel(const double* Z, int64_t ZS, int64_t r0, double* out, int64_t nrows, int64_t ldout, int d)
+{
+    const int64_t i = (int64_t)blockIdx.x * blockDim.x + threadIdx.x;
+    if (i >= nrows * d) return;
+    const int64_t r = i % nrows, p = i / nrows;
+    out[r + ldout * p] = Z[(r0 + r) * ZS + p];
+}
+
+__global__ void append_gathered_kernel(double* Z, int64_t ZS, int64_t M, const double* slab, int64_t n_loc,
+                                       int R, int d)
+{
+    const int64_t i = (int64_t)blockIdx.x * blockDim.x + threadIdx.x;
+    const int64_t per = n_loc * d;
+    if (i >= per * R) return;
+    const int64_t r = i / per, rem = i % per, p = rem / n_loc, j = rem % n_loc;
+    Z[(M + r * n_loc + j) * ZS + p] = slab[i];
+}
+
+__global__ void append_batch_kernel(double* Z, int64_t ZS, int64_t base, const double* slab, int64_t n_loc, int R, int cnt, int d)
+{
+    const int64_t i = (int64_t)blockIdx.x * blockDim.x + threadIdx.x;
+    const int64_t per = n_loc * d;
+    if (i >= per * cnt * R) return;
+    const int64_t r = i / (per * cnt), rem = i % (per * cnt), sidx = rem / per, rem2 = rem % per, p = rem2 / n_loc, j = rem2 % n_loc;
+    Z[(base + (sidx * R + r) * n_loc + j) * ZS + p] = slab[i];
+}
+
+__global__ void rhat_moments_kernel(const double* chain, int64_t N, int d, int64_t s0, int64_t n, int nchunk,
+                                    double* S1, double* S2)
 {
     const int64_t i = (int64_t)blockIdx.x * blockDim.x + threadIdx.x;
     if (i >= N * d) return;
-    const int h = blockIdx.y;
-    const int64_t stride = N * d;
+    rhat_moments_chunk(chain, N * d, i, (int)blockIdx.y, s0, n, nchunk, S1, S2);
+}
+
+__device__ __forceinline__ void rhat_chainstat(const double* chain, int64_t stride, int64_t i, int h, int64_t s0, int64_t n, int nchunk,
+                                               const double* S1, const double* S2, double& mean, double& s2)
+{
     const double x0 = chain[i + stride * (s0 + h * n)];
     double a = 0.0, b = 0.0;
     for (int ck = 0; ck < nchunk; ++ck) {
@@ -600,8 +609,21 @@
         b += S2[i + stride * (h * nchunk + ck)];
     }
     const double nn = (double)n;
-    mean_j[i + stride * h] = x0 + a / nn;
-    s2_j[i + stride * h] = (b - a * a / nn) / (nn - 1.0);
+    mean = x0 + a / nn;
+    s2 = (b - a * a / nn) / (nn - 1.0);
+}
+
+__global__ void rhat_chainstats_kernel(const double* chain, int64_t N, int d, int64_t s0, int64_t n, int nchunk,
+                                       const double* S1, const double* S2, double* mean_j, double* s2_j)
+{
+    const int64_t i = (int64_t)blockIdx.x * blockDim.x + threadIdx.x;
+    if (i >= N * d) return;
+    const int h = blockIdx.y;
+    const int64_t stride = N * d;
+    double mean, s2;
+    rhat_chainstat(chain, stride, i, h, s0, n, nchunk, S1, S2, mean, s2);
+    mean_j[i + stride * h] = mean;
+    s2_j[i + stride * h] = s2;
 }
 
 __global__ void __launch_bounds__(256) rhat_reduce_kernel(const double* mean_j, const double* s2_j, int64_t N, int d,
@@ -643,19 +665,16 @@
     }
 }
 
-__global__ void __launch_bounds__(256) rhat_tail_kernel(const double* mean_j, const double* s2_j, int64_t N, int d,
-                                                        double n, double m, double* rhat)
-{
-    __shared__ double ra[256], rb[256];
-    const int p = blockIdx.x;
-    const int64_t stride = N * d;
+template <class FM, class FS>
+__device__ __forceinline__ void rhat_tail_reduce(FM mean_of, FS s2_of, int64_t N, double n, double m, double* ra, double* rb, double* out)
+{
     double a = 0.0, b = 0.0;
     int64_t h0 = 0, c0 = threadIdx.x;
     while (c0 >= N) { c0 -= N; ++h0; }
     {
         int64_t h = h0, c = c0;
         for (int64_t k = threadIdx.x; k < 2 * N; k += 256) {
-            a += mean_j[c + N * p + stride * h];
+            a += mean_of(k, h, c);
             c += 256;
             while (c >= N) { c -= N; ++h; }
         }
@@ -672,10 +691,9 @@
     {
         int64_t h = h0, c = c0;
         for (int64_t k = threadIdx.x; k < 2 * N; k += 256) {
-            const int64_t at = c + N * p + stride * h;
-            const double dv = mean_j[at] - gm;
+            const double dv = mean_of(k, h, c) - gm;
             a = fma(dv, dv, a);
-            b += s2_j[at];
+            b += s2_of(k, h, c);
             c += 256;
             while (c >= N) { c -= N; ++h; }
         }
@@ -694,8 +712,36 @@
         const double B = n / (m - 1.0) * ra[0];
         const double W = rb[0] / m;
         const double varhat = (n - 1.0) / n * W + B / n;
-        rhat[p] = sqrt(varhat / W);
-    }
+        *out = sqrt(varhat / W);
+    }
+}
+
+__global__ void __launch_bounds__(256) rhat_tail_kernel(const double* mean_j, const double* s2_j, int64_t N, int d,
+                                                        double n, double m, double* rhat)
+{
+    __shared__ double ra[256], rb[256];
+    const int p = blockIdx.x;
+    const int64_t stride = N * d;
+    rhat_tail_reduce([&](int64_t, int64_t h, int64_t c) { return mean_j[c + N * p + stride * h]; },
+                     [&](int64_t, int64_t h, int64_t c) { return s2_j[c + N * p + stride * h]; }, N, n, m, ra, rb, rhat + p);
+}
+
+__global__ void __launch_bounds__(256) rhat_finish_kernel(const double* chain, int64_t N, int d, int64_t s0, int64_t n, int nchunk,
+                                                          const double* S1, const double* S2, double m, double* rhat)
+{
+    __shared__ double ra[256], rb[256];
+    extern __shared__ double sj[];
+    const int p = blockIdx.x;
+    const int64_t stride = N * d;
+    int64_t h = 0, c = threadIdx.x;
+    while (c >= N) { c -= N; ++h; }
+    for (int64_t k = threadIdx.x; k < 2 * N; k += 256) {
+        rhat_chainstat(chain, stride, c + N * p, (int)h, s0, n, nchunk, S1, S2, sj[k], sj[2 * N + k]);
+        c += 256;
+        while (c >= N) { c -= N; ++h; }
+    }
+    rhat_tail_reduce([&](int64_t k, int64_t, int64_t) { return sj[k]; },
+                     [&](int64_t k, int64_t, int64_t) { return sj[2 * N + k]; }, N, (double)n, m, ra, rb, rhat + p);
 }
 
 __global__ void rhat_final_kernel(const double* in, int d, double n, double m, double* rhat)
diff --git a/demc.jl_amd/csrc/demcz_kernels_ps.h b/demc.jl_amd/csrc/demcz_kernels_ps.h
--- a/demc.jl_amd/csrc/demcz_kernels_ps.h
+++ b/demc.jl_amd/csrc/demcz_kernels_ps.h
@@ -26,9 +26,9 @@
 constexpr int PRODUCE_WAVES = 4;
 constexpr size_t PRODUCE_THROTTLE_LDS = 64 * 1024;
 template <int D>
-__global__ void __launch_bounds__(64 * PRODUCE_WAVES) produce_kernel(const WindowParams P)
+__global__ void __launch_bounds__(64 * PRODUCE_WAVES) __attribute__((amdgpu_waves_per_eu(8))) produce_kernel(const WindowParams P)
 {
-    pc_produce<D>(P, (int64_t)blockIdx.x * PRODUCE_WAVES + (int64_t)(threadIdx.x >> 6), (int)(threadIdx.x & 63));
+    pc_produce<D, true>(P, (int64_t)blockIdx.x * PRODUCE_WAVES + (int64_t)(threadIdx.x >> 6), (int)(threadIdx.x & 63));
 }
 
 template <int TARGET, int D, bool LIVE, bool TEMPER>
diff --git a/demc.jl_amd/csrc/demcz_kernels_rec.h b/demc.jl_amd/csrc/demcz_kernels_rec.h
--- a/demc.jl_amd/csrc/demcz_kernels_rec.h
+++ b/demc.jl_amd/csrc/demcz_kernels_rec.h
@@ -35,28 +35,10 @@
 }
 
 template <int D>
-__device__ __forceinline__ void pc_produce(const WindowParams& P, int64_t pb, int lane = -1)
+__device__ __forceinline__ void pc_draw(const WindowParams& P, int64_t c, int role, int gi)
 {
-    if (lane < 0) lane = (int)threadIdx.x;
     constexpr int NPAIRS = (D == 1) ? 1 : (D + 1) / 2;
     constexpr int S = NPAIRS + 2;
-    int64_t c;
-    int role, gi;
-    if (produce_by_generation(P.rec_fields, P.next_ngen)) {
-        const int64_t gblocks = (P.next_ngen + 63) / 64;
-        const int64_t per_chain = (int64_t)S * gblocks;
-        c = pb / per_chain;
-        const int64_t rem = pb % per_chain;
-        role = (int)(rem / gblocks);
-        gi = (int)(rem % gblocks) * 64 + lane;
-    } else {
-        const int64_t nbc = (P.N + 63) / 64;
-        const int64_t plane = pb / nbc;
-        c = (pb % nbc) * 64 + lane;
-        role = (int)(plane % S);
-        gi = (int)(plane / S);
-    }
-    if (gi >= P.next_ngen || c >= P.N) return;
     philox_blocks rng;
     uint64_t r1, r2;
     rng.block(P.seed, (uint64_t)(P.chain_id0 + c), (uint64_t)(P.next_g_first + gi - 1) * (uint64_t)S + (uint64_t)role, r1, r2);
@@ -80,6 +62,38 @@
             const int p0 = (D == 1) ? 0 : 2 * (role - 1);
             rec[at(gi, p0)] = R * cs;
             if (p0 + 1 < D) rec[at(gi, p0 + 1)] = R * sn;
+        }
+    }
+}
+
+template <int D, bool MOMENTS = false>
+__device__ __forceinline__ void pc_produce(const WindowParams& P, int64_t pb, int lane = -1)
+{
+    if (lane < 0) lane = (int)threadIdx.x;
+    constexpr int NPAIRS = (D == 1) ? 1 : (D + 1) / 2;
+    constexpr int S = NPAIRS + 2;
+    int64_t c;
+    int role, gi;
+    if (produce_by_generation(P.rec_fields, P.next_ngen)) {
+        const int64_t gblocks = (P.next_ngen + 63) / 64;
+        const int64_t per_chain = (int64_t)S * gblocks;
+        c = pb / per_chain;
+        const int64_t rem = pb % per_chain;
+        role = (int)(rem / gblocks);
+        gi = (int)(rem % gblocks) * 64 + lane;
+    } else {
+        const int64_t nbc = (P.N + 63) / 64;
+        const int64_t plane = pb / nbc;
+        c = (pb % nbc) * 64 + lane;
+        role = (int)(plane % S);
+        gi = (int)(plane / S);
+    }
+    if (gi < P.next_ngen && c < P.N) pc_draw<D>(P, c, role, gi);
+    if constexpr (MOMENTS) {
+        if (P.mom_tasks > 0 && pb % P.mom_stride == 0 && pb / P.mom_stride < P.mom_tasks) {
+            const int64_t task = pb / P.mom_stride, nd = P.N * P.d, nblk = (nd + 63) / 64;
+            const int64_t i = (task % nblk) * 64 + lane;
+            if (i < nd) rhat_moments_chunk(P.mom_hist, nd, i, (int)(task / nblk), P.mom_s0, P.mom_n, P.mom_nchunk, P.mom_S1, P.mom_S2);
         }
     }
 }
diff --git a/demc.jl_amd/engine.py b/demc.jl_amd/engine.py
--- a/demc.jl_amd/engine.py
+++ b/demc.jl_amd/engine.py
@@ -157,6 +157,11 @@
                                             C.byref(n), _lib.ptr(mx), C.c_int32(n_max), _lib.ptr(last)))
         return int(g_stop.value), mx[:n.value].copy(), last
 
+    def checked_rhat(self, i: int):
+        r = np.full(self.d, np.nan)
+        self._chk(self._L.demcz_get_checked_rhat(self._h, C.c_int32(int(i)), _lib.ptr(r)))
+        return r
+
     def set_kernel_timing(self, enabled: bool):
         self._chk(self._L.demcz_set_kernel_timing(self._h, C.c_int32(1 if enabled else 0)))
 
@@ -195,6 +200,11 @@
         c = (C.c_int64 * 3)()
         self._chk(self._L.demcz_debug_kernel_counts(self._h, c))
         return dict(zip(("ps2", "ps_general", "other"), (int(v) for v in c)))
+
+    def check_counts(self):
+        k = (C.c_int64 * 2)()
+        self._chk(self._L.demcz_debug_check_counts(self._h, k))
+        return dict(zip(("fused", "standalone"), (int(v) for v in k)))
 
     def kernel_name(self):
         buf = C.create_string_buffer(192)
diff --git a/include/demcz.h b/include/demcz.h
--- a/include/demcz.h
+++ b/include/demcz.h
@@ -138,6 +138,8 @@
                           int64_t every, double threshold, int64_t* g_stop, int32_t* n_checks,
                           double* rhat_max, int32_t n_max, double* rhat_last);
 
+int32_t demcz_get_checked_rhat(demcz_handle* h, int32_t i, double* rhat);
+
 
 int32_t demcz_set_kernel_timing(demcz_handle* h, int32_t enabled);
 int32_t demcz_get_kernel_time(demcz_handle* h, int64_t* launches, double* milliseconds);
@@ -152,6 +154,7 @@
 int32_t demcz_set_live_rearms(demcz_handle* h, int32_t n);
 int32_t demcz_get_live_rearms(const demcz_handle* h, int32_t* rearms, int32_t* left);
 int32_t demcz_debug_kernel_counts(const demcz_handle* h, int64_t* counts);
+int32_t demcz_debug_check_counts(const demcz_handle* h, int64_t* counts);
 int32_t demcz_debug_kernel_name(const demcz_handle* h, char* buf, int32_t cap);
 
 int32_t demcz_debug_set_live_fault(demcz_handle* h, int32_t polls, int64_t g_from);
```

Result: no change. 690.3 million, median of 3 (+0.1%).
